# tusen-ai/SST

Hardware: AMD Instinct MI355X
Metric: LiDAR frames/sec (SST backbone fwd+bwd) at Waymo 0.32m voxels (higher is better)
Workload: dtype f32 (storage, accumulation, attention, LayerNorm, reductions: fp32; the dense products of the encoder layers from the EXACT three-way bf16 split of both fp32 operands, six bf16 MFMA products with fp32 accumulation - error vs float64 <= 2 x the fp32 matrix pipe's: tests/test_gpu_dense_f32x6.py)

## Files before the change

### include/sst_amd.h

```cpp
#ifndef SST_AMD_H
#define SST_AMD_H

#include <stdint.h>

#ifdef __cplusplus
extern "C" {
#endif

#define SST_OK 0
#define SST_ERR_ARG (-1)
#define SST_ERR_UNSUPPORTED (-2)
#define SST_ERR_KEYSPACE (-3)

typedef enum { SST_REDUCE_SUM = 0, SST_REDUCE_MEAN = 1, SST_REDUCE_MAX = 2 } sst_reduce_t;

const char* sst_version(void);

int sst_dynamic_voxelize_f32(const float* d_points, int64_t n, int64_t row_stride,
                             const float voxel_size[3], const float coors_range[6],
                             int32_t* d_coors, int64_t coors_stride, int coors_col0, int batch_idx,
                             void* stream);
void sst_dynamic_voxelize_grid(const float voxel_size[3], const float coors_range[6], int32_t grid_xyz[3]);

int64_t sst_scan_workspace_bytes(int64_t n);
int sst_exclusive_scan_i32(const int32_t* d_in, int32_t* d_out, int64_t n, int32_t* d_total,
                           void* d_workspace, void* stream);

int64_t sst_sort_workspace_bytes(int64_t n);
int sst_sort_pairs_u64(uint64_t* d_keys_in, uint64_t* d_keys_out, uint32_t* d_perm_out, int64_t n,
                       int key_bits, void* d_workspace, void* stream);

int64_t sst_unique_workspace_bytes(int64_t n);
int sst_unique_rows(const void* d_coors, int coor_is_i64, int64_t n, int ncols, int64_t row_stride,
                    const int64_t* h_mins, const int64_t* h_extents, int invalid_if_negative,
                    uint32_t* d_perm, int32_t* d_inverse, int32_t* d_offsets, uint64_t* d_ukeys,
                    int32_t* d_num_unique, void* d_workspace, void* stream);
int sst_unpack_keys(const uint64_t* d_ukeys, int64_t m, int ncols, const int64_t* h_mins,
                    const int64_t* h_extents, void* d_rows_out, int out_is_i64, int64_t out_stride,
                    int out_col0, void* stream);

int sst_segment_reduce_fwd_f32(const float* d_feats, int64_t n, int c, const uint32_t* d_perm,
                               const int32_t* d_offsets, const int32_t* d_group_index, int64_t m, int mode,
                               float* d_out, int32_t* d_argmax, const int32_t* d_m_limit, void* stream);
int64_t sst_segment_reduce_work_words(int64_t n, int64_t m, int c);
int sst_segment_reduce_fwd_work_f32(const float* d_feats, int64_t n, int c, const uint32_t* d_perm,
                                    const int32_t* d_offsets, const int32_t* d_group_index, int64_t m, int mode,
                                    float* d_out, int32_t* d_argmax, const int32_t* d_m_limit, int32_t* d_work,
                                    int64_t work_capacity, const float* d_scale, const float* d_shift, void* stream);
int64_t sst_segment_long_scratch_bytes(int64_t n, int64_t m, int c);
int sst_segment_reduce_long_f32(const float* d_feats, int64_t n, int c, const uint32_t* d_perm, const int32_t* d_inverse,
                                int inverse_shift, const int32_t* d_offsets, int64_t m, int mode, void* d_scratch,
                                float* d_out, int32_t* d_argmax, void* stream);
int sst_segment_reduce_profile_next(void* start, void* stop);
int sst_segment_reduce_bwd_f32(const float* d_grad_out, int64_t m, int c, const int32_t* d_inverse,
                               int inverse_shift, const int32_t* d_offsets, const int32_t* d_group_index,
                               const int32_t* d_argmax, int64_t n, int mode, float* d_grad_feats,
                               const int32_t* d_m_limit, void* stream);

int sst_concat_gather_f32(const float* d_x, int64_t ldx, int c1, const float* d_g, int64_t ldg, int c2,
                          const int32_t* d_idx, int64_t n, float* d_out, void* stream);

int sst_recover_bev_f32(const float* d_feats, int64_t ldf, const void* d_coors, int coor_is_i64, int64_t ldc, int64_t m,
                        int batch, int ny, int nx, int c, int32_t* d_cell_map, int32_t* d_cell_of_voxel, float* d_canvas,
                        void* stream);
int sst_recover_bev_bwd_f32(const float* d_grad_canvas, const int32_t* d_cell_of_voxel, int64_t m, int c,
                            float* d_grad_feats, void* stream);

int sst_vfe_decorate_f32(const float* d_points, int64_t ldp, int64_t n, int c, const int32_t* d_inverse,
                         const float* d_voxel_mean, int64_t ldm, float cluster_div, const void* d_coors,
                         int coor_is_i64, int64_t ldc, const float* voxel_size, const float* offsets,
                         int with_cluster, int with_center, float* d_out, int64_t ldo, void* stream);

int64_t sst_ingroup_rank_workspace_bytes(int64_t n);
int sst_ingroup_rank_i64(const int64_t* d_group, int64_t n, int key_bits, int64_t* d_rank,
                         void* d_workspace, void* stream);

int sst_window_coors(const void* d_coors, int coor_is_i64, int64_t m, const int32_t sparse_shape[3],
                     const int32_t window_shape[3], int32_t* d_win0, int32_t* d_ciw0,
                     int32_t* d_win1, int32_t* d_ciw1, void* stream);

int64_t sst_region_batching_workspace_bytes(int64_t m);
int sst_region_batching(const int32_t* d_win0, const int32_t* d_win1, int64_t m, int win_bits,
                        const int32_t* h_levels , int n_levels,
                        int32_t* d_keep, int32_t* d_newidx,
                        int32_t* d_level0, int32_t* d_level1, int32_t* d_inner0, int32_t* d_inner1,
                        int32_t* d_flat2win0, int32_t* d_flat2win1,
                        int32_t* d_tok0, int32_t* d_tok1, int32_t* d_winoff0, int32_t* d_winoff1,
                        int32_t* d_winlevel0, int32_t* d_winlevel1, int32_t* d_counts,
                        void* d_workspace, void* stream);
int sst_window_order_i32(const int32_t* d_winoff, int n_windows, int max_tokens, int32_t* d_order, void* stream);


int64_t sst_frame_windows_per_sample(const int32_t grid_zyx[3], const int32_t window_shape[3]);
int sst_frame_voxels_i32(const uint64_t* d_ukeys, const int32_t* d_inverse, const int32_t* d_num_groups, int64_t n_points, int batch_size, const int32_t grid_zyx[3],
                         int drop_mode, int32_t* d_vcoors, int32_t* d_gidx, int32_t* d_coors_map, int32_t* d_grid,
                         int32_t* d_counts, int32_t* d_dropped_groups, void* stream);
int64_t sst_window_plan_workspace_bytes(int64_t n_upper, int64_t n_windows);
int sst_window_plan_i32(const int32_t* d_vcoors, const int32_t* d_grid, int64_t n_upper, int batch_size,
                        const int32_t grid_zyx[3], const int32_t window_shape[3], const int32_t* h_levels, int n_levels,
                        uint32_t seed, int64_t* d_feat_index, int32_t* d_feat_index32, int64_t* d_out_coors,
                        int32_t* d_tok1, int32_t* d_winoff0, int32_t* d_winoff1, int32_t* d_posidx0, int32_t* d_posidx1,
                        int32_t* d_counts, void* d_workspace, void* stream);

int sst_sra_attn_fwd_f32(const float* d_q, const float* d_k, const float* d_v, int64_t ldq, int64_t ldk,
                         int64_t ldv, const int32_t* d_tok, const int32_t* d_winoff, int64_t n_windows,
                         int n_heads, float scale, int max_tokens, int impl, float* d_o, int64_t ldo,
                         float* d_lse, void* stream);
int64_t sst_sra_attn_bwd_workspace_bytes(int64_t n_tokens, int n_heads);
int sst_sra_attn_bwd_f32(const float* d_q, const float* d_k, const float* d_v, const float* d_o,
                         const float* d_do, const float* d_lse, int64_t ldq, int64_t ldk, int64_t ldv,
                         int64_t ldo, int64_t lddo, const int32_t* d_tok, const int32_t* d_winoff,
                         int64_t n_windows, int64_t n_tokens, int n_heads, float scale, int max_tokens,
                         int impl, float* d_dq, float* d_dk, float* d_dv, int64_t lddq, int64_t lddk,
                         int64_t lddv, void* d_workspace, void* stream);

int sst_sra_attn_fwd_ord_f32(const float* d_q, const float* d_k, const float* d_v, int64_t ldq, int64_t ldk, int64_t ldv,
                             const int32_t* d_tok, const int32_t* d_winoff, const int32_t* d_win_order, int64_t n_windows,
                             int n_heads, float scale, int max_tokens, int impl, float* d_o, int64_t ldo, float* d_lse,
                             void* stream);
int sst_sra_attn_bwd_ord_f32(const float* d_q, const float* d_k, const float* d_v, const float* d_o, const float* d_do,
                             const float* d_lse, int64_t ldq, int64_t ldk, int64_t ldv, int64_t ldo, int64_t lddo,
                             const int32_t* d_tok, const int32_t* d_winoff, const int32_t* d_win_order, int64_t n_windows,
                             int64_t n_tokens, int n_heads, float scale, int max_tokens, int impl, float* d_dq,
                             float* d_dk, float* d_dv, int64_t lddq, int64_t lddk, int64_t lddv, void* d_workspace,
                             void* stream);

int sst_sra_attn_cos_fwd_f32(const float* d_q, const float* d_k, const float* d_v, int64_t ldq, int64_t ldk, int64_t ldv,
                             const int32_t* d_tok, const int32_t* d_winoff, const int32_t* d_win_order, int64_t n_windows,
                             int n_heads, const float* d_head_scale, int max_tokens, float* d_o, int64_t ldo, float* d_lse,
                             void* stream);
int sst_sra_attn_cos_bwd_f32(const float* d_q, const float* d_k, const float* d_v, const float* d_o, const float* d_do,
                             const float* d_lse, int64_t ldq, int64_t ldk, int64_t ldv, int64_t ldo, int64_t lddo,
                             const int32_t* d_tok, const int32_t* d_winoff, const int32_t* d_win_order, int64_t n_windows,
                             int64_t n_tokens, int n_heads, const float* d_head_scale, int max_tokens, float* d_dq, float* d_dk,
                             float* d_dv, int64_t lddq, int64_t lddk, int64_t lddv, float* d_r, void* stream);

int sst_sra_attn_fwd_bf16(const void* d_q, const void* d_k, const void* d_v, int64_t ldq, int64_t ldk, int64_t ldv,
                          const int32_t* d_tok, const int32_t* d_winoff, int64_t n_windows, int n_heads, float scale,
                          int max_tokens, void* d_o, int64_t ldo, float* d_lse, void* stream);
int sst_sra_attn_bwd_bf16(const void* d_q, const void* d_k, const void* d_v, const void* d_o, const void* d_do,
                          const float* d_lse, int64_t ldq, int64_t ldk, int64_t ldv, int64_t ldo, int64_t lddo,
                          const int32_t* d_tok, const int32_t* d_winoff, int64_t n_windows, int n_heads, float scale,
                          int max_tokens, void* d_dq, void* d_dk, void* d_dv, int64_t lddq, int64_t lddk, int64_t lddv,
                          void* stream);
int sst_sra_attn_bf16_profile_next(int backward, void* start, void* stop);
int sst_sra_attn_fwd_ord_bf16(const void* d_q, const void* d_k, const void* d_v, int64_t ldq, int64_t ldk, int64_t ldv,
                              const int32_t* d_tok, const int32_t* d_winoff, const int32_t* d_win_order, int64_t n_windows,
                              int n_heads, float scale, int max_tokens, void* d_o, int64_t ldo, float* d_lse,
                              void* stream);
int sst_sra_attn_bwd_ord_bf16(const void* d_q, const void* d_k, const void* d_v, const void* d_o, const void* d_do,
                              const float* d_lse, int64_t ldq, int64_t ldk, int64_t ldv, int64_t ldo, int64_t lddo,
                              const int32_t* d_tok, const int32_t* d_winoff, const int32_t* d_win_order, int64_t n_windows,
                              int n_heads, float scale, int max_tokens, void* d_dq, void* d_dk, void* d_dv, int64_t lddq,
                              int64_t lddk, int64_t lddv, void* stream);
int sst_sra_attn_cos_fwd_bf16(const void* d_q, const void* d_k, const void* d_v, int64_t ldq, int64_t ldk, int64_t ldv,
                              const int32_t* d_tok, const int32_t* d_winoff, const int32_t* d_win_order, int64_t n_windows,
                              int n_heads, const float* d_head_scale, int max_tokens, void* d_o, int64_t ldo, float* d_lse,
                              void* stream);
int sst_sra_attn_cos_bwd_bf16(const void* d_q, const void* d_k, const void* d_v, const void* d_o, const void* d_do,
                              const float* d_lse, int64_t ldq, int64_t ldk, int64_t ldv, int64_t ldo, int64_t lddo,
                              const int32_t* d_tok, const int32_t* d_winoff, const int32_t* d_win_order, int64_t n_windows,
                              int n_heads, const float* d_head_scale, int max_tokens, void* d_dq, void* d_dk, void* d_dv,
                              int64_t lddq, int64_t lddk, int64_t lddv, float* d_r, void* stream);

int sst_add_layernorm_fwd_bf16(const void* d_x, const void* d_res, const float* d_weight, const float* d_bias, int64_t m,
                               int c, float eps, void* d_y, void* d_sum, float* d_stats, const float* d_pos_table,
                               const int32_t* d_pos_idx, void* d_y_plus_pos, void* stream);
int sst_add_layernorm_bwd_bf16(const void* d_dy, const void* d_dy2, const void* d_sum, const float* d_stats,
                               const float* d_weight, int64_t m, int c, void* d_dx, float* d_dweight, float* d_dbias,
                               void* d_workspace, void* stream);
int sst_cast_add_pos_bf16(const void* d_x, int x_is_bf16, int64_t m, int c, const float* d_pos_table,
                          const int32_t* d_pos_idx, void* d_out, void* stream);

int sst_tall_linear_bf16(const void* d_x, int64_t ldx, const void* d_w, const float* d_bias, int64_t m, int k, int n,
                         int epilogue, const void* d_aux_in, void* d_aux_out, int64_t ldaux, void* d_y, int64_t ldy,
                         void* stream);
int sst_tall_linear_bf16_partition(int64_t m, int k, int n, int epi_is_ln, int64_t* blocks, int64_t* rows_per_wave);
int sst_tall_linear_ln_bf16(const void* d_x, int64_t ldx, const void* d_w, const float* d_bias, int64_t m, int k,
                            const void* d_res, int64_t ldres, const float* d_ln_weight, const float* d_ln_bias, float eps,
                            void* d_y, void* d_sum, float* d_stats, const float* d_pos_table, const int32_t* d_pos_idx,
                            void* d_y_plus_pos, void* stream);
typedef struct sst_wgrad_problem_bf16 {
  const void* a;
  const void* b;
  int64_t lda, ldb, m;
// ... 12 lines not shown
int sst_cast_group_bf16(const sst_cast_problem_bf16* problems, int n, void* stream);

int sst_gather_rows_f32(const float* d_src, int64_t ld_src, const int32_t* d_idx, int64_t n_out, int c,
                        float fill, float* d_out, int64_t ld_out, void* stream);
int sst_add_table_rows_f32(const float* d_x, int64_t ldx, const float* d_table, int64_t ld_table, const int32_t* d_idx, int64_t m,
                           int c, float* d_out, int64_t ld_out, void* stream);
int sst_scatter_rows_f32(const float* d_src, int64_t ld_src, const int32_t* d_idx, int64_t n_src, int c,
                         float* d_out, int64_t ld_out, void* stream);

int sst_add_layernorm_act_fwd_f32(const float* d_x, const float* d_res, const float* d_weight, const float* d_bias,
                                  int64_t m, int c, float eps, int act, float* d_y, float* d_sum, float* d_stats,
                                  void* stream);
int sst_add_layernorm_act_bwd_f32(const float* d_dy, const float* d_sum, const float* d_stats, const float* d_weight,
                                  const float* d_bias, int act, int64_t m, int c, float* d_dx, float* d_dweight,
                                  float* d_dbias, void* d_workspace, void* stream);
int sst_add_layernorm_fwd_f32(const float* d_x, const float* d_res, const float* d_weight, const float* d_bias,
                              int64_t m, int c, float eps, float* d_y, float* d_sum, float* d_stats,
                              void* stream);
int sst_add_layernorm_pos_fwd_f32(const float* d_x, const float* d_res, const float* d_weight, const float* d_bias, int64_t m,
                                  int c, float eps, float* d_y, float* d_sum, float* d_stats, const float* d_pos_table,
                                  const int32_t* d_pos_idx, float* d_y_plus_pos, void* stream);
int64_t sst_add_layernorm_bwd_workspace_bytes(int64_t m, int c);
int sst_add_layernorm_bwd_f32(const float* d_dy, const float* d_sum, const float* d_stats,
                              const float* d_weight, int64_t m, int c, float* d_dx, float* d_dweight,
                              float* d_dbias, void* d_workspace, void* stream);
int64_t sst_colsum_workspace_bytes(int64_t m, int c);
int sst_colsum_f32(const float* d_x, int64_t m, int c, int64_t ld, float* d_out, void* d_workspace, void* stream);

int64_t sst_weight_grad_workspace_bytes(int64_t m, int out, int in);
int sst_weight_grad_f32(const float* d_dy, const float* d_x, int64_t m, int out, int in, int64_t ld_dy,
                        int64_t ld_x, float* d_dw, float* d_db, void* d_workspace, void* stream);
typedef struct sst_wgrad_problem_f32 {
  const float* dy;
  const float* x;
  int64_t m, ld_dy, ld_x;
  float* dw;
  float* db;
  int32_t out, in;
  const float* x_add_rows;
  const int32_t* x_add_index;
} sst_wgrad_problem_f32;
int64_t sst_weight_grad_group_workspace_bytes(const sst_wgrad_problem_f32* problems, int n);
int sst_weight_grad_group_f32(const sst_wgrad_problem_f32* problems, int n, void* d_workspace, void* stream);
int64_t sst_weight_grad_group_f32x6_workspace_bytes(const sst_wgrad_problem_f32* problems, int n);
int sst_weight_grad_group_f32x6(const sst_wgrad_problem_f32* problems, int n, void* d_workspace, void* stream);
int sst_weight_grad_group_f32x6_plan(const sst_wgrad_problem_f32* problems, int n, int* tiles, int* slices,
                                     int64_t* tokens_per_slice, int* lean_slices);

int64_t sst_bn_workspace_bytes(int64_t n, int c);
int sst_bn_stats_f32(const float* d_x, int64_t n, int c, int64_t ld, float* d_mean, float* d_var,
                     void* d_workspace, void* stream);
int sst_bn_act_fwd_f32(const float* d_x, int64_t n, int c, int64_t ldx, const float* d_scale,
                       const float* d_shift, int act, float* d_y, int64_t ldy, void* stream);
int sst_bn_act_bwd_reduce_f32(const float* d_dy, const float* d_x, int64_t n, int c, int64_t lddy, int64_t ldx,
                              const float* d_mean, const float* d_invstd, const float* d_scale,
                              const float* d_shift, int act, float* d_sum_g, float* d_sum_gxhat,
                              void* d_workspace, void* stream);
int sst_bn_act_bwd_apply_f32(const float* d_dy, const float* d_x, int64_t n, int c, int64_t lddy, int64_t ldx,
                             const float* d_mean, const float* d_invstd, const float* d_scale,
                             const float* d_shift, const float* d_coef_a, const float* d_coef_b, float coef_scale,
                             int act, float* d_dx, int64_t lddx, void* stream);
int sst_bn_prepare_f32(const float* d_x, int64_t n, int c, int64_t ld, const float* d_weight, const float* d_bias,
                       float eps, float* d_running_mean, float* d_running_var, float factor, float* d_out4,
                       void* d_workspace, void* stream);
int sst_bn_prepare_tracked_f32(const float* d_x, int64_t n, int c, int64_t ld, const float* d_weight,
                               const float* d_bias, float eps, float* d_running_mean, float* d_running_var,
                               float factor, int64_t* d_num_batches_tracked, float* d_out4, void* d_workspace,
                               void* stream);
int sst_vfe_linear_moments_f32(const float* d_x, int64_t ldx, int64_t n, int k, const float* d_w, int64_t ldw, int c,
                               float* d_y, int64_t ldy, void* d_workspace, void* stream);
int sst_bn_prepare_from_partials_f32(int64_t n, int c, const float* d_weight, const float* d_bias, float eps,
                                     float* d_running_mean, float* d_running_var, float factor,
                                     int64_t* d_num_batches_tracked, float* d_out4, void* d_workspace, void* stream);
int sst_bn_stats_from_partials_f32(int64_t n, int c, float* d_mean, float* d_var, void* d_workspace, void* stream);
int sst_bn_act_pool_bwd_reduce_f32(const float* d_dy, const float* d_x, int64_t n, int c, int64_t lddy, int64_t ldx,
                                   const float* d_mean, const float* d_invstd, const float* d_scale, const float* d_shift,
                                   int act, const int32_t* d_group, const int32_t* d_arg, const float* d_dpool, int64_t ldp,
                                   float* d_sum_g, float* d_sum_gxhat, void* d_workspace, void* stream);
int sst_bn_act_pool_bwd_apply_f32(const float* d_dy, const float* d_x, int64_t n, int c, int64_t lddy, int64_t ldx,
                                  const float* d_mean, const float* d_invstd, const float* d_scale, const float* d_shift,
                                  const float* d_coef_a, const float* d_coef_b, float coef_scale, int act,
                                  const int32_t* d_group, const int32_t* d_arg, const float* d_dpool, int64_t ldp, float* d_dx,
                                  int64_t lddx, void* stream);
int sst_bn_act_res_fwd_f32(const float* d_x, int64_t n, int c, int64_t ldx, const float* d_res, int64_t ldr,
                           const float* d_scale, const float* d_shift, int act, float* d_y, int64_t ldy, void* stream);
int sst_bn_act_res_bwd_reduce_f32(const float* d_dy, const float* d_x, const float* d_res, int64_t n, int c,
                                  int64_t lddy, int64_t ldx, int64_t ldr, const float* d_mean, const float* d_invstd,
                                  const float* d_scale, const float* d_shift, int act, float* d_sum_g,
                                  float* d_sum_gxhat, void* d_workspace, void* stream);
int sst_bn_act_res_bwd_apply_f32(const float* d_dy, const float* d_x, const float* d_res, int64_t n, int c,
                                 int64_t lddy, int64_t ldx, int64_t ldr, const float* d_mean, const float* d_invstd,
                                 const float* d_scale, const float* d_shift, const float* d_coef_a,
                                 const float* d_coef_b, float coef_scale, int act, float* d_dres, int64_t lddres,
                                 float* d_dx, int64_t lddx, void* stream);

int sst_tall_linear_f32(const float* d_x, int64_t ldx, const float* d_w, int64_t ldw, const float* d_bias,
                        int64_t m, int n, int k, int trans_w, int accumulate, float* d_y, int64_t ldy,
                        void* stream);
int sst_tall_linear_ln_f32(const float* d_x, int64_t ldx, const float* d_w, int64_t ldw, const float* d_bias, int64_t m, int k,
                           const float* d_res, int64_t ldres, const float* d_ln_weight, const float* d_ln_bias, float eps,
                           float* d_y, float* d_sum, float* d_stats, const float* d_pos_table, const int32_t* d_pos_idx,
                           float* d_y_plus_pos, void* stream);
int sst_tall_linear_epi_f32x3(const float* d_x, int64_t ldx, const float* d_w, int64_t ldw, int trans_w, const float* d_bias,
                              int64_t m, int k, int n, int epilogue, const float* d_aux_in, float* d_aux_out, int64_t ldaux,
                              float* d_y, int64_t ldy, void* stream);
int sst_tall_linear_ln_f32x3(const float* d_x, int64_t ldx, const float* d_w, int64_t ldw, const float* d_bias, int64_t m, int k,
                             const float* d_res, int64_t ldres, const float* d_ln_weight, const float* d_ln_bias, float eps,
                             float* d_y, float* d_sum, float* d_stats, const float* d_pos_table, const int32_t* d_pos_idx,
                             float* d_y_plus_pos, void* stream);
int sst_tall_linear_epi_f32x6(const float* d_x, int64_t ldx, const float* d_w, int64_t ldw, int trans_w, const float* d_bias,
                              int64_t m, int k, int n, int epilogue, const float* d_aux_in, float* d_aux_out, int64_t ldaux,
                              float* d_y, int64_t ldy, void* stream);
int sst_tall_linear_epi2_f32x6(const float* d_x, const float* d_x2, int x2_from_col, int64_t ldx, const float* d_w, int64_t ldw,
                               int trans_w, const float* d_bias, int64_t m, int k, int n, int epilogue, const float* d_aux_in,
                               float* d_aux_out, int64_t ldaux, float* d_y, int64_t ldy, void* stream);
int sst_tall_linear_add_rows_f32x6(const float* d_x, int64_t ldx, const float* d_w, int64_t ldw, int64_t m, int k, int n,
                                   const float* d_rows, int64_t ldrows, const int32_t* d_row_index, float* d_y, int64_t ldy,
                                   void* stream);
int sst_inproj_pos_f32x6(const float* d_x, int64_t ldx, const float* d_rows, const int32_t* d_index, const float* d_w, int64_t ldw,
                         const float* d_bias, int64_t m, float* d_y, int64_t ldy, void* stream);
int sst_tall_linear_f32x6_partition(int64_t m, int groups, int64_t* row_blocks, int64_t* rows_per_wave);
int sst_tall_linear_ln_f32x6(const float* d_x, int64_t ldx, const float* d_w, int64_t ldw, const float* d_bias, int64_t m, int k,
                             const float* d_res, int64_t ldres, const float* d_ln_weight, const float* d_ln_bias, float eps,
                             float* d_y, float* d_sum, float* d_stats, const float* d_pos_table, const int32_t* d_pos_idx,
                             float* d_y_plus_pos, void* stream);
int sst_add_layernorm_bwd2_f32(const float* d_dy, const float* d_dy2, const float* d_sum, const float* d_stats,
                               const float* d_weight, int64_t m, int c, float* d_dx, float* d_dweight, float* d_dbias,
                               void* d_workspace, void* stream);
typedef struct sst_encoder_layer_fwd_args {
  int64_t m, n_windows;
  int32_t n_heads, act, max_tokens, impl;
  float eps, scale;
  const float *x, *xp;
  const float *w_in, *b_in, *w_out, *b_out, *w1, *b1, *w2, *b2, *n1w, *n1b, *n2w, *n2b;
  const int32_t *tok, *winoff, *order;
  const float* pos_table;
  const int32_t* pos_idx;
  float *qkv, *o, *lse, *y1, *s1, *st1, *pre, *h, *s2, *y2, *st2, *y2p;
  const float* head_scale;
  void* wpack;
  const float* xpos_table;
  const int32_t* xpos_idx;
} sst_encoder_layer_fwd_args;
typedef struct sst_encoder_layer_bwd_args {
  int64_t m, n_windows;
  int32_t n_heads, act, max_tokens, impl;
  float eps, scale;
  const float *dy2, *dy2p;
  const float *x, *xp, *qkv, *o, *lse, *s1, *st1, *y1, *pre, *h, *s2, *st2;
  const float *w_in, *w_out, *w1, *w2, *n1w, *n2w;
  const int32_t *tok, *winoff, *order;
  float *ds2, *dpre, *ds1, *d_o, *dqkv;
  float *dw_in, *db_in, *dwo, *dbo, *dw1, *db1, *dw2, *db2, *dn1w, *dn1b, *dn2w, *dn2b;
  void* workspace;
  const float* head_scale;
  float* cos_r;
  float* dy1;
  const void* wpack;
  const float* xpos_table;
  const int32_t* xpos_idx;
} sst_encoder_layer_bwd_args;
int64_t sst_encoder_layer_bwd_workspace_bytes(int64_t m, int n_heads);
int64_t sst_encoder_layer_wpack_bytes(void);
int sst_encoder_layer_fwd_f32x6(const sst_encoder_layer_fwd_args* args, void* stream);
int sst_encoder_layer_bwd_f32x6(const sst_encoder_layer_bwd_args* args, void* stream);

// ... 733 lines not shown
```

### sst_amd/_lib.py

```python
import ctypes
import os
import subprocess

import torch

_HERE = os.path.dirname(os.path.abspath(__file__))
_CSRC = os.path.join(_HERE, 'csrc')
LIB_PATH = os.path.join(_CSRC, 'libsst_amd.so')

_lib = None

c_i64 = ctypes.c_int64
c_i32 = ctypes.c_int
c_f32 = ctypes.c_float
c_ptr = ctypes.c_void_p



class WgradProblemBF16(ctypes.Structure):
    _fields_ = [('a', c_ptr), ('b', c_ptr), ('lda', c_i64), ('ldb', c_i64), ('m', c_i64), ('out_w', c_ptr),
                ('out_b', c_ptr), ('p', ctypes.c_int32), ('bias_side', ctypes.c_int32),
                ('transpose_out', ctypes.c_int32), ('reserved', ctypes.c_int32)]


# ... 102 lines not shown
    + [(k, _I32 * 4) for k in ('q_inc', 'q_lo', 'q_hi')]
    + [('q_tag', ctypes.c_float * 4), ('lo', ctypes.c_float * 3), ('vs', ctypes.c_float * 3), ('grid', _I32 * 3)]))
IncrDeltaArgs = _struct('IncrDeltaArgs', 'sst_incr_delta_args of include/sst_amd.h', (
    [('base', ctypes.c_void_p * 8), ('n_base', c_i64 * 8), ('ld_base', c_i64 * 8), ('query', ctypes.c_void_p),
     ('n_query', c_i64), ('ld_query', c_i64), ('mask', ctypes.c_void_p), ('workspace', ctypes.c_void_p),
     ('workspace_bytes', c_i64), ('n_clouds', _I32), ('lower_bound', _I32), ('lo', ctypes.c_float * 3),
     ('vs', ctypes.c_float * 3), ('grid', _I32 * 3)]))
FrameTransformArgs = _struct('FrameTransformArgs', 'sst_frame_transform_args of include/sst_amd.h', (
    [('src', ctypes.c_void_p * 8), ('dst', ctypes.c_void_p * 8), ('n', c_i64 * 8), ('mat', (ctypes.c_float * 12) * 8),
     ('n_clouds', _I32), ('cols', _I32)]))
AugmentParams = _struct('AugmentParams', 'sst_augment_params of include/sst_amd.h', (
    [(k, _I32) for k in ('flip_h', 'flip_v', 'rotate', 'shuffle')]
    + [(k, ctypes.c_float) for k in ('cos', 'sin', 'scale', 'angle')]
    + [('trans', ctypes.c_float * 3), ('reserved', ctypes.c_float), ('range', ctypes.c_float * 6), ('seed', ctypes.c_uint64)]))
AugmentArgs = _struct('AugmentArgs', 'sst_augment_args of include/sst_amd.h', (
    [(k, ctypes.c_void_p) for k in ('points', 'row_offsets', 'n_pasted', 'block_offsets', 'params', 'planes', 'plane_offsets',
                                    'out', 'counts', 'workspace')]
    + [(k, c_i64) for k in ('workspace_bytes', 'n_total')]
    + [(k, _I32) for k in ('batch', 'cols', 'n_blocks', 'n_planes', 'norm_mask', 'reserved')]
    + [('norm_mean', ctypes.c_float * 8), ('norm_std', ctypes.c_float * 8)]))
AugmentBoxArgs = _struct('AugmentBoxArgs', 'sst_augment_box_args of include/sst_amd.h', (
    [(k, ctypes.c_void_p) for k in ('boxes', 'labels', 'box_offsets', 'params', 'boxes_out', 'labels_out', 'counts')]
    + [(k, _I32) for k in ('batch', 'cols', 'n_boxes', 'filter', 'always_rotate', 'reserved')]))
FgGroupOffsets = _struct('FgGroupOffsets', 'sst_fg_group_offsets of include/sst_amd.h', [('off', c_i64 * 33)])

_P = ctypes.c_void_p
EncoderLayerFwdArgs = _struct('EncoderLayerFwdArgs', 'sst_encoder_layer_fwd_args of include/sst_amd.h', (
    [('m', c_i64), ('n_windows', c_i64)] + [(k, ctypes.c_int32) for k in ('n_heads', 'act', 'max_tokens', 'impl')]
    + [('eps', ctypes.c_float), ('scale', ctypes.c_float)]
    + [(k, _P) for k in ('x', 'xp', 'w_in', 'b_in', 'w_out', 'b_out', 'w1', 'b1', 'w2', 'b2', 'n1w', 'n1b', 'n2w', 'n2b',
                         'tok', 'winoff', 'order', 'pos_table', 'pos_idx',
                         'qkv', 'o', 'lse', 'y1', 's1', 'st1', 'pre', 'h', 's2', 'y2', 'st2', 'y2p', 'head_scale', 'wpack',
                         'xpos_table', 'xpos_idx')]))
EncoderLayerBwdArgs = _struct('EncoderLayerBwdArgs', 'sst_encoder_layer_bwd_args of include/sst_amd.h', (
    [('m', c_i64), ('n_windows', c_i64)] + [(k, ctypes.c_int32) for k in ('n_heads', 'act', 'max_tokens', 'impl')]
    + [('eps', ctypes.c_float), ('scale', ctypes.c_float)]
    + [(k, _P) for k in ('dy2', 'dy2p', 'x', 'xp', 'qkv', 'o', 'lse', 's1', 'st1', 'y1', 'pre', 'h', 's2', 'st2',
                         'w_in', 'w_out', 'w1', 'w2', 'n1w', 'n2w', 'tok', 'winoff', 'order',
                         'ds2', 'dpre', 'ds1', 'd_o', 'dqkv',
                         'dw_in', 'db_in', 'dwo', 'dbo', 'dw1', 'db1', 'dw2', 'db2', 'dn1w', 'dn1b', 'dn2w', 'dn2b',
                         'workspace', 'head_scale', 'cos_r', 'dy1', 'wpack', 'xpos_table', 'xpos_idx')]))


EncoderTailFwdArgs = _struct('EncoderTailFwdArgs', 'sst_encoder_tail_fwd_args of include/sst_amd.h', (
    [('m', c_i64), ('act', ctypes.c_int32), ('reserved', ctypes.c_int32), ('eps', ctypes.c_float), ('reserved_f', ctypes.c_float)]
    + [(k, _P) for k in ('o', 'x', 'packed', 'b_out', 'b1', 'b2', 'n1w', 'n1b', 'n2w', 'n2b', 'pos_table', 'pos_idx',
                         's1', 'st1', 'y1', 'pre', 'h', 's2', 'st2', 'y2', 'y2p')]))
EncoderTailBwdArgs = _struct('EncoderTailBwdArgs', 'sst_encoder_tail_bwd_args of include/sst_amd.h', (
    [('m', c_i64), ('act', ctypes.c_int32), ('reserved', ctypes.c_int32)]
    + [(k, _P) for k in ('dy2', 'dy2p', 's2', 'st2', 'pre', 's1', 'st1', 'packed', 'n1w', 'n2w',
                         'ds2', 'dpre', 'ds1', 'd_o', 'dn2w', 'dn2b', 'dn1w', 'dn1b', 'workspace')]))

EncoderTailFwdBF16Args = _struct('EncoderTailFwdBF16Args', 'sst_encoder_tail_fwd_bf16_args of include/sst_amd.h', (
    [('m', c_i64), ('act', ctypes.c_int32), ('reserved', ctypes.c_int32), ('eps', ctypes.c_float), ('reserved_f', ctypes.c_float)]
    + [(k, _P) for k in ('o', 'x', 'packed', 'b_out', 'b1', 'b2', 'n1w', 'n1b', 'n2w', 'n2b', 'pos_table', 'pos_idx',
                         's1', 'st1', 'y1', 'pre', 'h', 's2', 'st2', 'y2', 'y2p')]))
EncoderTailBwdBF16Args = _struct('EncoderTailBwdBF16Args', 'sst_encoder_tail_bwd_bf16_args of include/sst_amd.h', (
    [('m', c_i64), ('act', ctypes.c_int32), ('reserved', ctypes.c_int32)]
    + [(k, _P) for k in ('dy2', 'dy2p', 's2', 'st2', 'pre', 's1', 'st1', 'packed', 'n1w', 'n2w',
                         'ds2', 'dpre', 'ds1', 'd_o', 'dn2w', 'dn2b', 'dn1w', 'dn1b', 'workspace')]))


EncoderLayerFwdBF16Args = _struct('EncoderLayerFwdBF16Args', 'sst_encoder_layer_fwd_bf16_args of include/sst_amd.h', (
    [('m', c_i64), ('n_windows', c_i64)] + [(k, ctypes.c_int32) for k in ('n_heads', 'act', 'max_tokens', 'reserved')]
    + [('eps', ctypes.c_float), ('scale', ctypes.c_float)]
    + [(k, _P) for k in ('x', 'xp', 'wqk', 'wv', 'wout', 'w1', 'w2', 'b_in', 'b_out', 'b1', 'b2', 'n1w', 'n1b', 'n2w', 'n2b',
                         'tok', 'winoff', 'order', 'pos_table', 'pos_idx',
                         'qk', 'v', 'o', 'lse', 'y1', 's1', 'st1', 'pre', 'h', 's2', 'st2', 'y2', 'y2p', 'head_scale', 'wpack')]))
EncoderLayerBwdBF16Args = _struct('EncoderLayerBwdBF16Args', 'sst_encoder_layer_bwd_bf16_args of include/sst_amd.h', (
    [('m', c_i64), ('n_windows', c_i64)] + [(k, ctypes.c_int32) for k in ('n_heads', 'act', 'max_tokens', 'reserved')]
    + [('eps', ctypes.c_float), ('scale', ctypes.c_float)]
    + [(k, _P) for k in ('dy2', 'dy2p', 'x', 'xp', 'qk', 'v', 'o', 'lse', 's1', 'st1', 'y1', 'pre', 'h', 's2', 'st2',
                         'wqk_t', 'wv_t', 'wout_t', 'w1_t', 'w2_t', 'n1w', 'n2w', 'tok', 'winoff', 'order',
                         'ds2', 'dpre', 'dy1', 'ds1', 'd_o', 'dqkv', 'dxp', 'dx',
                         'dw_in', 'db_in', 'dwo', 'dbo', 'dw1', 'db1', 'dw2', 'db2', 'dn1w', 'dn1b', 'dn2w', 'dn2b',
                         'workspace', 'head_scale', 'cos_r', 'wpack')]))


_SIGNATURES = {
    'sst_version': (ctypes.c_char_p, []),
    'sst_dynamic_voxelize_f32': (c_i32, [c_ptr, c_i64, c_i64, c_ptr, c_ptr, c_ptr, c_i64, c_i32, c_i32, c_ptr]),
    'sst_dynamic_voxelize_grid': (None, [c_ptr, c_ptr, c_ptr]),
    'sst_scan_workspace_bytes': (c_i64, [c_i64]),
    'sst_exclusive_scan_i32': (c_i32, [c_ptr, c_ptr, c_i64, c_ptr, c_ptr, c_ptr]),
    'sst_sort_workspace_bytes': (c_i64, [c_i64]),
    'sst_sort_pairs_u64': (c_i32, [c_ptr, c_ptr, c_ptr, c_i64, c_i32, c_ptr, c_ptr]),
    'sst_unique_workspace_bytes': (c_i64, [c_i64]),
    'sst_unique_rows': (c_i32, [c_ptr, c_i32, c_i64, c_i32, c_i64, c_ptr, c_ptr, c_i32,
                                c_ptr, c_ptr, c_ptr, c_ptr, c_ptr, c_ptr, c_ptr]),
    'sst_unpack_keys': (c_i32, [c_ptr, c_i64, c_i32, c_ptr, c_ptr, c_ptr, c_i32, c_i64, c_i32, c_ptr]),
    'sst_segment_reduce_fwd_f32': (c_i32, [c_ptr, c_i64, c_i32, c_ptr, c_ptr, c_ptr, c_i64, c_i32, c_ptr, c_ptr,
                                           c_ptr, c_ptr]),
    'sst_encoder_layer_bwd_workspace_bytes': (c_i64, [c_i64, c_i32]),
    'sst_tall_linear_f32x6_partition': (c_i32, [c_i64, c_i32, c_ptr, c_ptr]),
    'sst_inproj_pos_f32x6': (c_i32, [c_ptr, c_i64, c_ptr, c_ptr, c_ptr, c_i64, c_ptr, c_i64, c_ptr, c_i64, c_ptr]),
    'sst_encoder_layer_wpack_bytes': (c_i64, []),
    'sst_encoder_layer_fwd_f32x6': (c_i32, [c_ptr, c_ptr]),
    'sst_encoder_layer_bwd_f32x6': (c_i32, [c_ptr, c_ptr]),
    'sst_encoder_tail_pack_bytes': (c_i64, []),
    'sst_encoder_tail_pack_f32x6': (c_i32, [c_ptr, c_ptr, c_ptr, c_ptr, c_ptr]),
    'sst_encoder_tail_pack_f32x6_many': (c_i32, [c_ptr, c_ptr, c_ptr, c_ptr, c_i32, c_ptr]),
    'sst_encoder_tail_bwd_workspace_bytes': (c_i64, [c_i64]),
    'sst_encoder_tail_fwd_f32x6': (c_i32, [c_ptr, c_ptr]),
    'sst_encoder_tail_bwd_f32x6': (c_i32, [c_ptr, c_ptr]),
    'sst_encoder_tail_pack_bf16_bytes': (c_i64, []),
    'sst_encoder_tail_pack_bf16': (c_i32, [c_ptr, c_ptr, c_ptr, c_ptr, c_ptr]),
    'sst_encoder_tail_pack_bf16_many': (c_i32, [c_ptr, c_ptr, c_ptr, c_ptr, c_i32, c_ptr]),
    'sst_encoder_tail_bwd_bf16_workspace_bytes': (c_i64, [c_i64]),
    'sst_encoder_tail_fwd_bf16': (c_i32, [c_ptr, c_ptr]),
    'sst_encoder_tail_bwd_bf16': (c_i32, [c_ptr, c_ptr]),
    'sst_encoder_layer_bwd_bf16_workspace_bytes': (c_i64, [c_i64]),
    'sst_encoder_layer_fwd_bf16': (c_i32, [c_ptr, c_ptr]),
    'sst_encoder_layer_bwd_bf16': (c_i32, [c_ptr, c_ptr]),
    'sst_segment_reduce_work_words': (c_i64, [c_i64, c_i64, c_i32]),
    'sst_segment_reduce_fwd_work_f32': (c_i32, [c_ptr, c_i64, c_i32, c_ptr, c_ptr, c_ptr, c_i64, c_i32, c_ptr, c_ptr,
                                                c_ptr, c_ptr, c_i64, c_ptr, c_ptr, c_ptr]),
    'sst_vfe_linear_moments_f32': (c_i32, [c_ptr, c_i64, c_i64, c_i32, c_ptr, c_i64, c_i32, c_ptr, c_i64, c_ptr, c_ptr]),
    'sst_bn_prepare_from_partials_f32': (c_i32, [c_i64, c_i32, c_ptr, c_ptr, c_f32, c_ptr, c_ptr, c_f32, c_ptr, c_ptr, c_ptr,
                                                 c_ptr]),
    'sst_bn_stats_from_partials_f32': (c_i32, [c_i64, c_i32, c_ptr, c_ptr, c_ptr, c_ptr]),
    'sst_bn_act_pool_bwd_reduce_f32': (c_i32, [c_ptr, c_ptr, c_i64, c_i32, c_i64, c_i64, c_ptr, c_ptr, c_ptr, c_ptr, c_i32,
                                               c_ptr, c_ptr, c_ptr, c_i64, c_ptr, c_ptr, c_ptr, c_ptr]),
    'sst_bn_act_pool_bwd_apply_f32': (c_i32, [c_ptr, c_ptr, c_i64, c_i32, c_i64, c_i64, c_ptr, c_ptr, c_ptr, c_ptr, c_ptr,
                                              c_ptr, c_f32, c_i32, c_ptr, c_ptr, c_ptr, c_i64, c_ptr, c_i64, c_ptr]),
    'sst_tall_linear_add_rows_f32x6': (c_i32, [c_ptr, c_i64, c_ptr, c_i64, c_i64, c_i32, c_i32, c_ptr, c_i64, c_ptr, c_ptr,
                                               c_i64, c_ptr]),
    'sst_segment_long_scratch_bytes': (c_i64, [c_i64, c_i64, c_i32]),
    'sst_segment_reduce_long_f32': (c_i32, [c_ptr, c_i64, c_i32, c_ptr, c_ptr, c_i32, c_ptr, c_i64, c_i32, c_ptr, c_ptr, c_ptr,
                                            c_ptr]),
    'sst_segment_reduce_profile_next': (c_i32, [c_ptr, c_ptr]),
    'sst_segment_reduce_bwd_f32': (c_i32, [c_ptr, c_i64, c_i32, c_ptr, c_i32, c_ptr, c_ptr, c_ptr, c_i64, c_i32,
                                           c_ptr, c_ptr, c_ptr]),
    'sst_ingroup_rank_workspace_bytes': (c_i64, [c_i64]),
    'sst_ingroup_rank_i64': (c_i32, [c_ptr, c_i64, c_i32, c_ptr, c_ptr, c_ptr]),
    'sst_window_coors': (c_i32, [c_ptr, c_i32, c_i64, c_ptr, c_ptr, c_ptr, c_ptr, c_ptr, c_ptr, c_ptr]),
    'sst_window_order_i32': (c_i32, [c_ptr, c_i32, c_i32, c_ptr, c_ptr]),
    'sst_region_batching_workspace_bytes': (c_i64, [c_i64]),
    'sst_region_batching': (c_i32, [c_ptr, c_ptr, c_i64, c_i32, c_ptr, c_i32] + [c_ptr] * 15 + [c_ptr, c_ptr]),
    'sst_frame_windows_per_sample': (c_i64, [c_ptr, c_ptr]),
    'sst_frame_voxels_i32': (c_i32, [c_ptr, c_ptr, c_ptr, c_i64, c_i32, c_ptr, c_i32, c_ptr, c_ptr, c_ptr, c_ptr,
                                     c_ptr, c_ptr, c_ptr]),
    'sst_window_plan_workspace_bytes': (c_i64, [c_i64, c_i64]),
    'sst_window_plan_i32': (c_i32, [c_ptr, c_ptr, c_i64, c_i32, c_ptr, c_ptr, c_ptr, c_i32, ctypes.c_uint32] + [c_ptr] * 11),
    'sst_sra_attn_fwd_f32': (c_i32, [c_ptr, c_ptr, c_ptr, c_i64, c_i64, c_i64, c_ptr, c_ptr, c_i64, c_i32,
                                     c_f32, c_i32, c_i32, c_ptr, c_i64, c_ptr, c_ptr]),
    'sst_sra_attn_bwd_f32': (c_i32, [c_ptr] * 6 + [c_i64] * 5 + [c_ptr, c_ptr, c_i64, c_i64, c_i32, c_f32,
                                                                 c_i32, c_i32, c_ptr, c_ptr, c_ptr,
                                                                 c_i64, c_i64, c_i64, c_ptr, c_ptr]),
    'sst_sra_attn_fwd_ord_f32': (c_i32, [c_ptr, c_ptr, c_ptr, c_i64, c_i64, c_i64, c_ptr, c_ptr, c_ptr, c_i64, c_i32,
                                         c_f32, c_i32, c_i32, c_ptr, c_i64, c_ptr, c_ptr]),
    'sst_sra_attn_bwd_ord_f32': (c_i32, [c_ptr] * 6 + [c_i64] * 5 + [c_ptr, c_ptr, c_ptr, c_i64, c_i64, c_i32, c_f32,
                                                                     c_i32, c_i32, c_ptr, c_ptr, c_ptr,
                                                                     c_i64, c_i64, c_i64, c_ptr, c_ptr]),
    'sst_sra_attn_bwd_workspace_bytes': (c_i64, [c_i64, c_i32]),
    'sst_sra_attn_cos_fwd_f32': (c_i32, [c_ptr, c_ptr, c_ptr, c_i64, c_i64, c_i64, c_ptr, c_ptr, c_ptr, c_i64, c_i32,
                                         c_ptr, c_i32, c_ptr, c_i64, c_ptr, c_ptr]),
    'sst_sra_attn_cos_bwd_f32': (c_i32, [c_ptr] * 6 + [c_i64] * 5 + [c_ptr, c_ptr, c_ptr, c_i64, c_i64, c_i32, c_ptr,
                                                                     c_i32, c_ptr, c_ptr, c_ptr,
                                                                     c_i64, c_i64, c_i64, c_ptr, c_ptr]),
    'sst_sra_attn_fwd_bf16': (c_i32, [c_ptr, c_ptr, c_ptr, c_i64, c_i64, c_i64, c_ptr, c_ptr, c_i64, c_i32, c_f32, c_i32,
                                      c_ptr, c_i64, c_ptr, c_ptr]),
    'sst_sra_attn_bwd_bf16': (c_i32, [c_ptr] * 6 + [c_i64] * 5 + [c_ptr, c_ptr, c_i64, c_i32, c_f32, c_i32, c_ptr, c_ptr,
                                                                  c_ptr, c_i64, c_i64, c_i64, c_ptr]),
    'sst_sra_attn_bf16_profile_next': (c_i32, [c_i32, c_ptr, c_ptr]),
    'sst_sra_attn_fwd_ord_bf16': (c_i32, [c_ptr, c_ptr, c_ptr, c_i64, c_i64, c_i64, c_ptr, c_ptr, c_ptr, c_i64, c_i32, c_f32,
                                          c_i32, c_ptr, c_i64, c_ptr, c_ptr]),
    'sst_sra_attn_bwd_ord_bf16': (c_i32, [c_ptr] * 6 + [c_i64] * 5 + [c_ptr, c_ptr, c_ptr, c_i64, c_i32, c_f32, c_i32, c_ptr,
                                                                      c_ptr, c_ptr, c_i64, c_i64, c_i64, c_ptr]),
    'sst_sra_attn_cos_fwd_bf16': (c_i32, [c_ptr, c_ptr, c_ptr, c_i64, c_i64, c_i64, c_ptr, c_ptr, c_ptr, c_i64, c_i32, c_ptr,
                                          c_i32, c_ptr, c_i64, c_ptr, c_ptr]),
    'sst_sra_attn_cos_bwd_bf16': (c_i32, [c_ptr] * 6 + [c_i64] * 5 + [c_ptr, c_ptr, c_ptr, c_i64, c_i32, c_ptr, c_i32, c_ptr,
                                                                      c_ptr, c_ptr, c_i64, c_i64, c_i64, c_ptr, c_ptr]),
    'sst_add_layernorm_fwd_bf16': (c_i32, [c_ptr, c_ptr, c_ptr, c_ptr, c_i64, c_i32, c_f32, c_ptr, c_ptr, c_ptr, c_ptr,
                                           c_ptr, c_ptr, c_ptr]),
    'sst_add_layernorm_bwd_bf16': (c_i32, [c_ptr, c_ptr, c_ptr, c_ptr, c_ptr, c_i64, c_i32, c_ptr, c_ptr, c_ptr, c_ptr,
                                           c_ptr]),
    'sst_cast_add_pos_bf16': (c_i32, [c_ptr, c_i32, c_i64, c_i32, c_ptr, c_ptr, c_ptr, c_ptr]),
    'sst_weight_grad_group_workspace_bytes': (c_i64, [c_ptr, c_i32]),
    'sst_weight_grad_group_f32': (c_i32, [c_ptr, c_i32, c_ptr, c_ptr]),
    'sst_weight_grad_group_f32x6_workspace_bytes': (c_i64, [c_ptr, c_i32]),
    'sst_weight_grad_group_f32x6': (c_i32, [c_ptr, c_i32, c_ptr, c_ptr]),
    'sst_weight_grad_group_f32x6_plan': (c_i32, [c_ptr, c_i32, c_ptr, c_ptr, c_ptr, c_ptr]),
    'sst_tall_linear_ln_f32': (c_i32, [c_ptr, c_i64, c_ptr, c_i64, c_ptr, c_i64, c_i32, c_ptr, c_i64, c_ptr, c_ptr, c_f32, c_ptr,
                                       c_ptr, c_ptr, c_ptr, c_ptr, c_ptr, c_ptr]),
    'sst_tall_linear_ln_f32x3': (c_i32, [c_ptr, c_i64, c_ptr, c_i64, c_ptr, c_i64, c_i32, c_ptr, c_i64, c_ptr, c_ptr, c_f32, c_ptr,
                                         c_ptr, c_ptr, c_ptr, c_ptr, c_ptr, c_ptr]),
    'sst_tall_linear_epi_f32x3': (c_i32, [c_ptr, c_i64, c_ptr, c_i64, c_i32, c_ptr, c_i64, c_i32, c_i32, c_i32, c_ptr, c_ptr,
                                          c_i64, c_ptr, c_i64, c_ptr]),
    'sst_tall_linear_ln_f32x6': (c_i32, [c_ptr, c_i64, c_ptr, c_i64, c_ptr, c_i64, c_i32, c_ptr, c_i64, c_ptr, c_ptr, c_f32, c_ptr,
                                         c_ptr, c_ptr, c_ptr, c_ptr, c_ptr, c_ptr]),
    'sst_tall_linear_epi_f32x6': (c_i32, [c_ptr, c_i64, c_ptr, c_i64, c_i32, c_ptr, c_i64, c_i32, c_i32, c_i32, c_ptr, c_ptr,
                                          c_i64, c_ptr, c_i64, c_ptr]),
    'sst_tall_linear_epi2_f32x6': (c_i32, [c_ptr, c_ptr, c_i32, c_i64, c_ptr, c_i64, c_i32, c_ptr, c_i64, c_i32, c_i32, c_i32,
                                           c_ptr, c_ptr, c_i64, c_ptr, c_i64, c_ptr]),
    'sst_add_layernorm_bwd2_f32': (c_i32, [c_ptr, c_ptr, c_ptr, c_ptr, c_ptr, c_i64, c_i32, c_ptr, c_ptr, c_ptr, c_ptr, c_ptr]),
    'sst_tall_linear_epi_f32': (c_i32, [c_ptr, c_i64, c_ptr, c_i64, c_i32, c_ptr, c_i64, c_i32, c_i32, c_i32, c_ptr, c_ptr,
                                        c_i64, c_ptr, c_i64, c_ptr]),
    'sst_tall_linear_bf16': (c_i32, [c_ptr, c_i64, c_ptr, c_ptr, c_i64, c_i32, c_i32, c_i32, c_ptr, c_ptr, c_i64, c_ptr,
                                     c_i64, c_ptr]),
    'sst_tall_linear_bf16_partition': (c_i32, [c_i64, c_i32, c_i32, c_i32, c_ptr, c_ptr]),
    'sst_tall_linear_ln_bf16': (c_i32, [c_ptr, c_i64, c_ptr, c_ptr, c_i64, c_i32, c_ptr, c_i64, c_ptr, c_ptr, c_f32, c_ptr, c_ptr,
                                        c_ptr, c_ptr, c_ptr, c_ptr, c_ptr]),
    'sst_wgrad_group_workspace_bytes': (c_i64, [c_ptr, c_i32]),
    'sst_wgrad_group_bf16': (c_i32, [c_ptr, c_i32, c_ptr, c_ptr]),
    'sst_cast_group_bf16': (c_i32, [c_ptr, c_i32, c_ptr]),
    'sst_gather_rows_f32': (c_i32, [c_ptr, c_i64, c_ptr, c_i64, c_i32, c_f32, c_ptr, c_i64, c_ptr]),
    'sst_add_table_rows_f32': (c_i32, [c_ptr, c_i64, c_ptr, c_i64, c_ptr, c_i64, c_i32, c_ptr, c_i64, c_ptr]),
    'sst_scatter_rows_f32': (c_i32, [c_ptr, c_i64, c_ptr, c_i64, c_i32, c_ptr, c_i64, c_ptr]),
    'sst_add_layernorm_fwd_f32': (c_i32, [c_ptr, c_ptr, c_ptr, c_ptr, c_i64, c_i32, c_f32, c_ptr, c_ptr, c_ptr,
                                          c_ptr]),
    'sst_add_layernorm_bwd_workspace_bytes': (c_i64, [c_i64, c_i32]),
    'sst_add_layernorm_pos_fwd_f32': (c_i32, [c_ptr, c_ptr, c_ptr, c_ptr, c_i64, c_i32, c_f32, c_ptr, c_ptr, c_ptr, c_ptr, c_ptr,
                                              c_ptr, c_ptr]),
    'sst_add_layernorm_act_fwd_f32': (c_i32, [c_ptr, c_ptr, c_ptr, c_ptr, c_i64, c_i32, c_f32, c_i32, c_ptr, c_ptr, c_ptr,
                                              c_ptr]),
    'sst_add_layernorm_act_bwd_f32': (c_i32, [c_ptr, c_ptr, c_ptr, c_ptr, c_ptr, c_i32, c_i64, c_i32, c_ptr, c_ptr, c_ptr,
                                              c_ptr, c_ptr]),
    'sst_add_layernorm_bwd_f32': (c_i32, [c_ptr, c_ptr, c_ptr, c_ptr, c_i64, c_i32, c_ptr, c_ptr, c_ptr, c_ptr,
                                          c_ptr]),
    'sst_weight_grad_workspace_bytes': (c_i64, [c_i64, c_i32, c_i32]),
    'sst_weight_grad_f32': (c_i32, [c_ptr, c_ptr, c_i64, c_i32, c_i32, c_i64, c_i64, c_ptr, c_ptr, c_ptr, c_ptr]),
    'sst_colsum_workspace_bytes': (c_i64, [c_i64, c_i32]),
    'sst_colsum_f32': (c_i32, [c_ptr, c_i64, c_i32, c_i64, c_ptr, c_ptr, c_ptr]),
    'sst_tall_linear_f32': (c_i32, [c_ptr, c_i64, c_ptr, c_i64, c_ptr, c_i64, c_i32, c_i32, c_i32, c_i32, c_ptr, c_i64,
                                    c_ptr]),
    'sst_tall_linear_gelu_f32': (c_i32, [c_ptr, c_i64, c_ptr, c_i64, c_ptr, c_i64, c_i32, c_i32, c_i32, c_i32, c_ptr, c_ptr,
# ... 319 lines not shown
```

### sst_amd/csrc/bn.hip

```cpp
#include "common.h"

namespace {

constexpr int kBnThreads = 256;

struct bn_pool_grad {
  const int32_t* group;
  const int32_t* arg;
  const float* dpool;
  int64_t ldp;
};
__device__ __forceinline__ float4 bn_pool_part(const bn_pool_grad& pg, int64_t row, int c, int cc) {
  float4 g = make_float4(0.f, 0.f, 0.f, 0.f);
  const int v = pg.group[row];
  if (v >= 0) {
    const int4 a = *(const int4*)(pg.arg + (int64_t)v * c + cc * 4);
    const float4 d = *(const float4*)(pg.dpool + (int64_t)v * pg.ldp + cc * 4);
    g.x = a.x == (int)row ? d.x : 0.f;
    g.y = a.y == (int)row ? d.y : 0.f;
    g.z = a.z == (int)row ? d.z : 0.f;
    g.w = a.w == (int)row ? d.w : 0.f;
  }
  return g;
}
// ... 134 lines not shown
    out[3 * c + ch] = sh;
    if (running_mean != nullptr) running_mean[ch] = (1.f - factor) * running_mean[ch] + factor * mean;
    if (running_var != nullptr) running_var[ch] = (1.f - factor) * running_var[ch] + factor * (var * unbiased);
    if (tracked != nullptr && ch == 0) tracked[0] += 1;
  }
}

__global__ __launch_bounds__(kBnThreads) void bn_act_fwd_k(const float* __restrict__ x, int64_t n, int c, int64_t ldx,
                                                          const float* __restrict__ scale,
                                                          const float* __restrict__ shift, int act,
                                                          const float* __restrict__ res, int64_t ldr,
                                                          float* __restrict__ y, int64_t ldy) {
  const int c4 = c >> 2;
  const int64_t total = n * c4;
  for (int64_t i = (int64_t)blockIdx.x * kBnThreads + threadIdx.x; i < total; i += (int64_t)gridDim.x * kBnThreads) {
    const int64_t row = i / c4;
    const int cc = (int)(i - row * c4);
    const float4 v = *(const float4*)(x + row * ldx + cc * 4);
    const float4 sc = *(const float4*)(scale + cc * 4);
    const float4 sh = *(const float4*)(shift + cc * 4);
    float4 o = make_float4(v.x * sc.x + sh.x, v.y * sc.y + sh.y, v.z * sc.z + sh.z, v.w * sc.w + sh.w);
    if (res != nullptr) {
      const float4 r = *(const float4*)(res + row * ldr + cc * 4);
      o.x += r.x, o.y += r.y, o.z += r.z, o.w += r.w;
    }
    if (act) {
      o.x = o.x > 0.f ? o.x : 0.f;
      o.y = o.y > 0.f ? o.y : 0.f;
      o.z = o.z > 0.f ? o.z : 0.f;
      o.w = o.w > 0.f ? o.w : 0.f;
    }
    *(float4*)(y + row * ldy + cc * 4) = o;
  }
}

__global__ __launch_bounds__(kBnThreads) void bn_act_bwd_k(const float* __restrict__ dy, const float* __restrict__ x,
                                                          int64_t n, int c, int64_t lddy, int64_t ldx,
                                                          const float* __restrict__ mean,
                                                          const float* __restrict__ invstd,
                                                          const float* __restrict__ scale,
                                                          const float* __restrict__ shift,
                                                          const float* __restrict__ ca, const float* __restrict__ cb,
                                                          float coef_scale, int act, const float* __restrict__ res,
                                                          int64_t ldr, float* __restrict__ dres, int64_t lddres,
                                                          float* __restrict__ dx, int64_t lddx, const bn_pool_grad pg) {
  const int c4 = c >> 2;
  const int64_t total = n * c4;
  for (int64_t i = (int64_t)blockIdx.x * kBnThreads + threadIdx.x; i < total; i += (int64_t)gridDim.x * kBnThreads) {
    const int64_t row = i / c4;
    const int cc = (int)(i - row * c4);
    const float4 v = *(const float4*)(x + row * ldx + cc * 4);
    float4 g = make_float4(0.f, 0.f, 0.f, 0.f);
    if (dy != nullptr) g = *(const float4*)(dy + row * lddy + cc * 4);
    if (pg.group != nullptr) {
      const float4 sp = bn_pool_part(pg, row, c, cc);
      g.x += sp.x, g.y += sp.y, g.z += sp.z, g.w += sp.w;
    }
    const float4 sc = *(const float4*)(scale + cc * 4);
    const float4 sh = *(const float4*)(shift + cc * 4);
    const float4 mu = *(const float4*)(mean + cc * 4);
    const float4 is = *(const float4*)(invstd + cc * 4);
    float4 a = *(const float4*)(ca + cc * 4);
    float4 b = *(const float4*)(cb + cc * 4);
    a.x *= coef_scale, a.y *= coef_scale, a.z *= coef_scale, a.w *= coef_scale;
    b.x *= coef_scale, b.y *= coef_scale, b.z *= coef_scale, b.w *= coef_scale;
    if (act) {
      float4 r = make_float4(0.f, 0.f, 0.f, 0.f);
      if (res != nullptr) r = *(const float4*)(res + row * ldr + cc * 4);
      g.x = (v.x * sc.x + sh.x + r.x) > 0.f ? g.x : 0.f;
      g.y = (v.y * sc.y + sh.y + r.y) > 0.f ? g.y : 0.f;
      g.z = (v.z * sc.z + sh.z + r.z) > 0.f ? g.z : 0.f;
      g.w = (v.w * sc.w + sh.w + r.w) > 0.f ? g.w : 0.f;
    }
    if (dres != nullptr) *(float4*)(dres + row * lddres + cc * 4) = g;
    float4 o;
    o.x = sc.x * (g.x - a.x - (v.x - mu.x) * is.x * b.x);
    o.y = sc.y * (g.y - a.y - (v.y - mu.y) * is.y * b.y);
    o.z = sc.z * (g.z - a.z - (v.z - mu.z) * is.z * b.z);
    o.w = sc.w * (g.w - a.w - (v.w - mu.w) * is.w * b.w);
    *(float4*)(dx + row * lddx + cc * 4) = o;
  }
}

__global__ __launch_bounds__(kBnThreads) void vfe_linear_smallk_k(const float* __restrict__ x, int64_t ldx, int64_t n, int k,
                                                                 const float* __restrict__ w, int64_t ldw, int c,
                                                                 float* __restrict__ y, int64_t ldy, int64_t rows_per_block,
                                                                 double* __restrict__ partial) {
  extern __shared__ __attribute__((aligned(16))) double red[];
  const int c4 = c >> 2;
  const int rpi = kBnThreads / c4;
  float* wt = (float*)(red + (size_t)rpi * 2 * c);
  for (int i = threadIdx.x; i < k * c; i += kBnThreads) {
    const int kk = i / c, ch = i - kk * c;
    wt[i] = w[(int64_t)ch * ldw + kk];
  }
  __syncthreads();
  const int ry = threadIdx.x / c4, cx = threadIdx.x - ry * c4;
  const int64_t beg = (int64_t)blockIdx.x * rows_per_block;
  const int64_t end = beg + rows_per_block < n ? beg + rows_per_block : n;
  double s1[4] = {0., 0., 0., 0.}, s2[4] = {0., 0., 0., 0.};
  if (ry < rpi) {
    for (int64_t row = beg + ry; row < end; row += rpi) {
      const float* xr = x + row * ldx;
      float4 acc = make_float4(0.f, 0.f, 0.f, 0.f);
      for (int kk = 0; kk < k; ++kk) {
        const float xv = xr[kk];
        const float4 wv = *(const float4*)(wt + kk * c + cx * 4);
        acc.x = fmaf(xv, wv.x, acc.x), acc.y = fmaf(xv, wv.y, acc.y), acc.z = fmaf(xv, wv.z, acc.z), acc.w = fmaf(xv, wv.w, acc.w);
      }
      *(float4*)(y + row * ldy + cx * 4) = acc;
      s1[0] += acc.x, s1[1] += acc.y, s1[2] += acc.z, s1[3] += acc.w;
      s2[0] += (double)acc.x * acc.x, s2[1] += (double)acc.y * acc.y;
      s2[2] += (double)acc.z * acc.z, s2[3] += (double)acc.w * acc.w;
    }
#pragma unroll
    for (int q = 0; q < 4; ++q) {
      red[(size_t)ry * 2 * c + cx * 4 + q] = s1[q];
      red[(size_t)ry * 2 * c + c + cx * 4 + q] = s2[q];
    }
  }
  __syncthreads();
  double* dst = partial + (int64_t)blockIdx.x * 2 * c;
  for (int i = threadIdx.x; i < 2 * c; i += kBnThreads) {
    double t = 0.;
    for (int r = 0; r < rpi; ++r) t += red[(size_t)r * 2 * c + i];
    dst[i] = t;
  }
}

int moments_grid(int64_t n, int64_t* rows_per_block) {
  int64_t rpb = 128;
  int64_t grid = sst_div_up(n, rpb);
  if (grid > 512) {
    rpb = sst_div_up(n, 512);
    grid = sst_div_up(n, rpb);
  }
  *rows_per_block = rpb;
  return (int)grid;
}

bool bn_shape_ok(int64_t n, int c) { return n >= 0 && c >= 4 && (c & 3) == 0 && c <= 1024; }

}

extern "C" {

int64_t sst_bn_workspace_bytes(int64_t n, int c) {
  (void)n;
  return (int64_t)1024 * 2 * c * sizeof(double) + 256;
}

int sst_bn_stats_f32(const float* d_x, int64_t n, int c, int64_t ld, float* d_mean, float* d_var, void* d_workspace,
                     void* stream) {
  if (!bn_shape_ok(n, c) || ld < c || (ld & 3)) return SST_ERR_UNSUPPORTED;
  if (n == 0) return SST_ERR_ARG;
  if (!d_x || !d_mean || !d_var || !d_workspace || ((uintptr_t)d_x & 15)) return SST_ERR_ARG;
  hipStream_t st = (hipStream_t)stream;
  int64_t rpb;
  const int grid = moments_grid(n, &rpb);
  double* partial = (double*)d_workspace;
  const size_t lds = (size_t)kBnThreads * 8 * sizeof(double);
  hipLaunchKernelGGL(bn_moments_k<0>, dim3(grid), dim3(kBnThreads), lds, st, d_x, nullptr, n, c, ld, 0, nullptr,
                     nullptr, nullptr, nullptr, 0, nullptr, 0, rpb, partial, bn_pool_grad{nullptr, nullptr, nullptr, 0});
  hipLaunchKernelGGL(bn_finish_k<0>, dim3((c + 31) / 32), dim3(1024), 0, st, partial, grid, c, 1.0 / (double)n,
                     d_mean, d_var);
  SST_LAUNCH_CHECK();
// ... 129 lines not shown
  const int rpi = kBnThreads / (c >> 2);
  const size_t lds = (size_t)rpi * 2 * c * sizeof(double) + (size_t)k * c * sizeof(float);
  hipLaunchKernelGGL(vfe_linear_smallk_k, dim3(grid), dim3(kBnThreads), lds, (hipStream_t)stream, d_x, ldx, n, k, d_w, ldw, c,
                     d_y, ldy, rpb, (double*)d_workspace);
  SST_LAUNCH_CHECK();
  return SST_OK;
}

int sst_bn_prepare_from_partials_f32(int64_t n, int c, const float* d_weight, const float* d_bias, float eps,
                                     float* d_running_mean, float* d_running_var, float factor,
                                     int64_t* d_num_batches_tracked, float* d_out4, void* d_workspace, void* stream) {
  if (!bn_shape_ok(n, c)) return SST_ERR_UNSUPPORTED;
  if (n == 0 || !d_out4 || !d_workspace) return SST_ERR_ARG;
  int64_t rpb;
  const int grid = moments_grid(n, &rpb);
  const float unbiased = n > 1 ? (float)((double)n / (double)(n - 1)) : 1.f;
  hipLaunchKernelGGL(bn_prepare_finish_k, dim3((c + 31) / 32), dim3(1024), 0, (hipStream_t)stream, (const double*)d_workspace,
                     grid, c, 1.0 / (double)n, d_weight, d_bias, eps, d_running_mean, d_running_var, factor, unbiased,
                     d_num_batches_tracked, d_out4);
  SST_LAUNCH_CHECK();
  return SST_OK;
}

int sst_bn_stats_from_partials_f32(int64_t n, int c, float* d_mean, float* d_var, void* d_workspace, void* stream) {
  if (!bn_shape_ok(n, c)) return SST_ERR_UNSUPPORTED;
  if (n == 0 || !d_mean || !d_var || !d_workspace) return SST_ERR_ARG;
  int64_t rpb;
  const int grid = moments_grid(n, &rpb);
  hipLaunchKernelGGL(bn_finish_k<0>, dim3((c + 31) / 32), dim3(1024), 0, (hipStream_t)stream, (const double*)d_workspace, grid,
                     c, 1.0 / (double)n, d_mean, d_var);
  SST_LAUNCH_CHECK();
  return SST_OK;
}

int sst_bn_act_pool_bwd_reduce_f32(const float* d_dy, const float* d_x, int64_t n, int c, int64_t lddy, int64_t ldx,
                                   const float* d_mean, const float* d_invstd, const float* d_scale, const float* d_shift,
                                   int act, const int32_t* d_group, const int32_t* d_arg, const float* d_dpool, int64_t ldp,
                                   float* d_sum_g, float* d_sum_gxhat, void* d_workspace, void* stream) {
  if (!bn_shape_ok(n, c) || ldx < c || (ldx & 3) || act < 0 || act > 1 || ldp < c || (ldp & 3)) return SST_ERR_UNSUPPORTED;
  if (d_dy && (lddy < c || (lddy & 3) || ((uintptr_t)d_dy & 15))) return SST_ERR_UNSUPPORTED;
  if (!d_sum_g || !d_sum_gxhat) return SST_ERR_ARG;
  hipStream_t st = (hipStream_t)stream;
  if (n == 0) {
    SST_HIP(hipMemsetAsync(d_sum_g, 0, sizeof(float) * c, st));
    SST_HIP(hipMemsetAsync(d_sum_gxhat, 0, sizeof(float) * c, st));
    return SST_OK;
  }
  if (!d_x || !d_mean || !d_invstd || !d_scale || !d_shift || !d_workspace || !d_group || !d_arg || !d_dpool ||
      ((uintptr_t)d_x & 15) || ((uintptr_t)d_arg & 15) || ((uintptr_t)d_dpool & 15))
    return SST_ERR_ARG;
  int64_t rpb;
  const int grid = moments_grid(n, &rpb);
  double* partial = (double*)d_workspace;
  const size_t lds = (size_t)kBnThreads * 8 * sizeof(double);
  hipLaunchKernelGGL(bn_moments_k<1>, dim3(grid), dim3(kBnThreads), lds, st, d_x, d_dy, n, c, ldx, lddy, d_mean, d_invstd,
                     d_scale, d_shift, act, nullptr, 0, rpb, partial, bn_pool_grad{d_group, d_arg, d_dpool, ldp});
  hipLaunchKernelGGL(bn_finish_k<1>, dim3((c + 31) / 32), dim3(1024), 0, st, partial, grid, c, 0.0, d_sum_g, d_sum_gxhat);
  SST_LAUNCH_CHECK();
  return SST_OK;
}

int sst_bn_act_pool_bwd_apply_f32(const float* d_dy, const float* d_x, int64_t n, int c, int64_t lddy, int64_t ldx,
                                  const float* d_mean, const float* d_invstd, const float* d_scale, const float* d_shift,
                                  const float* d_coef_a, const float* d_coef_b, float coef_scale, int act,
                                  const int32_t* d_group, const int32_t* d_arg, const float* d_dpool, int64_t ldp, float* d_dx,
                                  int64_t lddx, void* stream) {
  if (!bn_shape_ok(n, c) || ldx < c || lddx < c || (ldx & 3) || (lddx & 3) || act < 0 || act > 1 || ldp < c || (ldp & 3))
    return SST_ERR_UNSUPPORTED;
  if (d_dy && (lddy < c || (lddy & 3) || ((uintptr_t)d_dy & 15))) return SST_ERR_UNSUPPORTED;
  if (n == 0) return SST_OK;
  if (!d_x || !d_mean || !d_invstd || !d_scale || !d_shift || !d_coef_a || !d_coef_b || !d_dx || !d_group || !d_arg ||
      !d_dpool || ((uintptr_t)d_x & 15) || ((uintptr_t)d_dx & 15) || ((uintptr_t)d_arg & 15) || ((uintptr_t)d_dpool & 15))
    return SST_ERR_ARG;
  const int64_t total = n * (c >> 2);
  int64_t grid = sst_div_up(total, kBnThreads);
  if (grid > 8192) grid = 8192;
  hipLaunchKernelGGL(bn_act_bwd_k, dim3((unsigned)grid), dim3(kBnThreads), 0, (hipStream_t)stream, d_dy, d_x, n, c, lddy, ldx,
                     d_mean, d_invstd, d_scale, d_shift, d_coef_a, d_coef_b, coef_scale, act, nullptr, 0, nullptr, 0, d_dx, lddx,
                     bn_pool_grad{d_group, d_arg, d_dpool, ldp});
  SST_LAUNCH_CHECK();
  return SST_OK;
}

}
```

### sst_amd/csrc/frame_plan.hip

```cpp
#include "common.h"

namespace {

struct fp_geom {
  int B, gz, gy, gx;
  int wx, wy, wz;
  int nwx, nwy, nwz;
  int sh[2][3];
  int n_levels;
  int cap[8], lo[8], hi[8];
};

__device__ __forceinline__ void fp_decode(uint64_t key, const fp_geom& G, int& b, int& z, int& y, int& x) {
  uint64_t k = key - 1;
  x = (int)(k % (uint64_t)(G.gx + 1)) - 1;
  k /= (uint64_t)(G.gx + 1);
  y = (int)(k % (uint64_t)(G.gy + 1)) - 1;
  k /= (uint64_t)(G.gy + 1);
  z = (int)(k % (uint64_t)(G.gz + 1)) - 1;
  b = (int)(k / (uint64_t)(G.gz + 1));
}

__device__ int fp_lower_bound(const uint64_t* __restrict__ ukeys, int m_all, uint64_t key) {
  int lo = 0, hi = m_all;
// ... 171 lines not shown
          const bool kp = vox[q] >= 0 && rank[q] < cap;
          const uint64_t bal = __ballot(kp);
          if (kp) inner[vox[q]] = run + __popcll(bal & lt);
          run += __popcll(bal);
        }
      }
    }
    if (lane == 0) cntk[w] = kept;
  }
}


__global__ __launch_bounds__(1024) void fp_window_scan_k(const int32_t* __restrict__ cntk0,
                                                         const int32_t* __restrict__ cntk1, int n_win,
                                                         int32_t* __restrict__ tokbase0, int32_t* __restrict__ tokbase1,
                                                         int32_t* __restrict__ winoff0, int32_t* __restrict__ winoff1,
                                                         int32_t* __restrict__ d_counts) {
  __shared__ int wsum[16], wsum2[16];
  __shared__ int smax;
  const int s = blockIdx.x;
  const int32_t* cnt = s ? cntk1 : cntk0;
  int32_t* tokbase = s ? tokbase1 : tokbase0;
  int32_t* winoff = s ? winoff1 : winoff0;
  const int tid = threadIdx.x, wave = tid >> 6, lane = tid & 63;
  if (tid == 0) smax = 0;
  int carry_tok = 0, carry_win = 0, my_max = 0;
  for (int base = 0; base < n_win; base += 1024) {
    const int w = base + tid;
    const int c = w < n_win ? cnt[w] : 0;
    const int ne = c > 0 ? 1 : 0;
    my_max = c > my_max ? c : my_max;
    const int ic = sst_wave_incl_scan(c);
    const int in = sst_wave_incl_scan(ne);
    if (lane == 63) {
      wsum[wave] = ic;
      wsum2[wave] = in;
    }
    __syncthreads();
    int off_c = 0, off_n = 0, tot_c = 0, tot_n = 0;
#pragma unroll
    for (int k = 0; k < 16; ++k) {
      const int a = wsum[k], bq = wsum2[k];
      if (k < wave) {
        off_c += a;
        off_n += bq;
      }
      tot_c += a;
      tot_n += bq;
    }
    __syncthreads();
    const int tb = carry_tok + off_c + ic - c;
    const int cw = carry_win + off_n + in - ne;
    if (w < n_win) {
      tokbase[w] = tb;
      if (ne) winoff[cw] = tb;
    }
    carry_tok += tot_c;
    carry_win += tot_n;
  }
  atomicMax(&smax, my_max);
  __syncthreads();
  if (tid == 0) {
    winoff[carry_win] = carry_tok;
    d_counts[2 + s] = carry_win;
    d_counts[4 + s] = smax;
    if (s == 0) d_counts[1] = carry_tok;
  }
}

__device__ __forceinline__ void fp_window_of(const fp_geom& G, int s, int b, int z, int y, int x, int& w, int& pos) {
  const int xs = x + G.sh[s][0], ys = y + G.sh[s][1], zs = z + G.sh[s][2];
  const int wxi = xs / G.wx, wyi = ys / G.wy, wzi = zs / G.wz;
  w = b * (G.nwx * G.nwy * G.nwz) + wxi * G.nwy * G.nwz + wyi * G.nwz + wzi;
  pos = ((zs - wzi * G.wz) * G.wy + (ys - wyi * G.wy)) * G.wx + (xs - wxi * G.wx);
}

__global__ __launch_bounds__(256) void fp_fill_k(const int32_t* __restrict__ vcoors, const int32_t* __restrict__ d_counts,
                                                 fp_geom G, const int32_t* __restrict__ keep,
                                                 const int32_t* __restrict__ inner0, const int32_t* __restrict__ inner1,
                                                 const int32_t* __restrict__ tokbase0,
                                                 const int32_t* __restrict__ tokbase1, int64_t* __restrict__ feat_index,
                                                 int32_t* __restrict__ feat_index32,
                                                 int64_t* __restrict__ out_coors, int32_t* __restrict__ tok1,
                                                 int32_t* __restrict__ posidx0, int32_t* __restrict__ posidx1) {
  const int m = d_counts[0];
  for (int v = blockIdx.x * blockDim.x + threadIdx.x; v < m; v += gridDim.x * blockDim.x) {
    if (keep[v] == 0) continue;
    const int b = vcoors[4 * v], z = vcoors[4 * v + 1], y = vcoors[4 * v + 2], x = vcoors[4 * v + 3];
    int w0, p0, w1, p1;
    fp_window_of(G, 0, b, z, y, x, w0, p0);
    fp_window_of(G, 1, b, z, y, x, w1, p1);
    const int ni = tokbase0[w0] + inner0[v];
    feat_index[ni] = v;
    feat_index32[ni] = v;
    out_coors[4 * (int64_t)ni + 0] = b;
    out_coors[4 * (int64_t)ni + 1] = z;
    out_coors[4 * (int64_t)ni + 2] = y;
    out_coors[4 * (int64_t)ni + 3] = x;
    posidx0[ni] = p0;
    posidx1[ni] = p1;
    tok1[tokbase1[w1] + inner1[v]] = ni;
  }
}

int fill_geom(fp_geom* G, int batch_size, const int32_t grid_zyx[3], const int32_t window_shape[3],
              const int32_t* h_levels, int n_levels) {
  if (batch_size < 1 || batch_size > 64 || !grid_zyx || !window_shape) return SST_ERR_ARG;
  G->B = batch_size;
  G->gz = grid_zyx[0];
  G->gy = grid_zyx[1];
  G->gx = grid_zyx[2];
  G->wx = window_shape[0];
  G->wy = window_shape[1];
  G->wz = window_shape[2];
  if (G->gz < 1 || G->gy < 1 || G->gx < 1 || G->wx < 1 || G->wy < 1 || G->wz < 1) return SST_ERR_ARG;
  if ((int64_t)G->wx * G->wy * G->wz > 512) return SST_ERR_UNSUPPORTED;
  if ((int64_t)G->B * G->gz * G->gy * G->gx > ((int64_t)1 << 28)) return SST_ERR_UNSUPPORTED;
  G->nwx = (G->gx + G->wx - 1) / G->wx + 1;
  G->nwy = (G->gy + G->wy - 1) / G->wy + 1;
  G->nwz = (G->gz + G->wz - 1) / G->wz + 1;
  G->sh[0][0] = G->wx;
  G->sh[0][1] = G->wy;
  G->sh[0][2] = G->wz;
  G->sh[1][0] = G->wx / 2;
  G->sh[1][1] = G->wy / 2;
  G->sh[1][2] = G->wz / 2;
  if (G->gz == G->wz) G->sh[0][2] = G->sh[1][2] = 0;
  G->n_levels = n_levels;
  for (int l = 0; l < 8; ++l) {
    G->cap[l] = (h_levels && l < n_levels) ? h_levels[3 * l + 0] : 0;
    G->lo[l] = (h_levels && l < n_levels) ? h_levels[3 * l + 1] : 0;
    G->hi[l] = (h_levels && l < n_levels) ? h_levels[3 * l + 2] : 0;
  }
  return SST_OK;
}

}

extern "C" {

int64_t sst_frame_windows_per_sample(const int32_t grid_zyx[3], const int32_t window_shape[3]) {
  fp_geom G;
  if (fill_geom(&G, 1, grid_zyx, window_shape, nullptr, 0) != SST_OK) return -1;
  return (int64_t)G.nwx * G.nwy * G.nwz;
}

int sst_frame_voxels_i32(const uint64_t* d_ukeys, const int32_t* d_inverse, const int32_t* d_num_groups, int64_t n_points, int batch_size, const int32_t grid_zyx[3],
                         int drop_mode, int32_t* d_vcoors, int32_t* d_gidx, int32_t* d_coors_map, int32_t* d_grid,
                         int32_t* d_counts, int32_t* d_dropped_groups, void* stream) {
  if (n_points < 0 || (drop_mode != 0 && drop_mode != 1)) return SST_ERR_ARG;
  const int32_t win1[3] = {1, 1, 1};
  fp_geom G;
  int rc = fill_geom(&G, batch_size, grid_zyx, win1, nullptr, 0);
  if (rc != SST_OK) return rc;
  if (!d_counts || !d_grid) return SST_ERR_ARG;
  hipStream_t st = (hipStream_t)stream;
  SST_HIP(hipMemsetAsync(d_counts, 0, 8 * sizeof(int32_t), st));
  SST_HIP(hipMemsetAsync(d_grid, 0xff, sizeof(int32_t) * (size_t)G.B * G.gz * G.gy * G.gx, st));
  if (d_dropped_groups) SST_HIP(hipMemsetAsync(d_dropped_groups, 0xff, sizeof(int32_t) * (size_t)G.B, st));
  if (n_points == 0) return SST_OK;
  if (!d_ukeys || !d_inverse || !d_num_groups || !d_vcoors || !d_gidx || !d_coors_map) return SST_ERR_ARG;
  if (n_points > 0x7fffffff) return SST_ERR_UNSUPPORTED;
  hipLaunchKernelGGL(fp_voxels_k, dim3(sst_grid_1d(n_points, 256)), dim3(256), 0, st, d_ukeys, d_inverse, (int)n_points,
                     d_num_groups, G, drop_mode, d_vcoors, d_gidx, d_coors_map, d_grid, d_counts, d_dropped_groups);
  SST_LAUNCH_CHECK();
  return SST_OK;
}

int64_t sst_window_plan_workspace_bytes(int64_t n_upper, int64_t n_windows) {
  const int64_t n = n_upper > 0 ? n_upper : 1, w = n_windows > 0 ? n_windows : 1;
  return 4 * sst_align_up(4 * n, 256) + 4 * sst_align_up(4 * (w + 1), 256);
}

int sst_window_plan_i32(const int32_t* d_vcoors, const int32_t* d_grid, int64_t n_upper, int batch_size,
                        const int32_t grid_zyx[3], const int32_t window_shape[3], const int32_t* h_levels, int n_levels,
                        uint32_t seed, int64_t* d_feat_index, int32_t* d_feat_index32, int64_t* d_out_coors,
                        int32_t* d_tok1,
                        int32_t* d_winoff0, int32_t* d_winoff1, int32_t* d_posidx0, int32_t* d_posidx1,
                        int32_t* d_counts, void* d_workspace, void* stream) {
  if (n_upper < 0 || n_levels < 1 || n_levels > 8 || !h_levels) return SST_ERR_ARG;
  fp_geom G;
  int rc = fill_geom(&G, batch_size, grid_zyx, window_shape, h_levels, n_levels);
  if (rc != SST_OK) return rc;
  if (n_upper == 0) return SST_OK;
  if (!d_vcoors || !d_grid || !d_feat_index || !d_feat_index32 || !d_out_coors || !d_tok1 || !d_winoff0 || !d_winoff1 || !d_posidx0 ||
      !d_posidx1 || !d_counts || !d_workspace)
    return SST_ERR_ARG;
  if (n_upper >= ((int64_t)1 << 30)) return SST_ERR_UNSUPPORTED;
  hipStream_t st = (hipStream_t)stream;
  const int n_win = G.B * G.nwx * G.nwy * G.nwz;
  sst_carver cv(d_workspace);
  int32_t* keep_a = cv.take<int32_t>(n_upper);
  int32_t* keep = cv.take<int32_t>(n_upper);
  int32_t* inner0 = cv.take<int32_t>(n_upper);
  int32_t* inner1 = cv.take<int32_t>(n_upper);
  int32_t* cntk0 = cv.take<int32_t>(n_win + 1);
  int32_t* cntk1 = cv.take<int32_t>(n_win + 1);
  int32_t* tokbase0 = cv.take<int32_t>(n_win + 1);
  int32_t* tokbase1 = cv.take<int32_t>(n_win + 1);
  SST_HIP(hipMemsetAsync(keep_a, 0, 2 * sst_align_up(4 * n_upper, 256), st));
  const dim3 wgrid((unsigned)((n_win + 3) / 4));
  hipLaunchKernelGGL(fp_window_pass_k<0>, wgrid, dim3(256), 0, st, d_grid, G, seed, (const int32_t*)nullptr, keep_a,
                     (int32_t*)nullptr, (int32_t*)nullptr);
  hipLaunchKernelGGL(fp_window_pass_k<1>, wgrid, dim3(256), 0, st, d_grid, G, seed, keep_a, keep, inner1, cntk1);
  hipLaunchKernelGGL(fp_window_pass_k<2>, wgrid, dim3(256), 0, st, d_grid, G, seed, keep, (int32_t*)nullptr, inner0,
                     cntk0);
  hipLaunchKernelGGL(fp_window_scan_k, dim3(2), dim3(1024), 0, st, cntk0, cntk1, n_win, tokbase0, tokbase1, d_winoff0,
                     d_winoff1, d_counts);
  hipLaunchKernelGGL(fp_fill_k, dim3(sst_grid_1d(n_upper, 256)), dim3(256), 0, st, d_vcoors, d_counts, G, keep, inner0,
                     inner1, tokbase0, tokbase1, d_feat_index, d_feat_index32, d_out_coors, d_tok1, d_posidx0, d_posidx1);
  SST_LAUNCH_CHECK();
  return SST_OK;
}

}
```

### sst_amd/csrc/sort_scan.hip

```cpp
#include "common.h"

namespace {

constexpr int kScanThreads = 256;
constexpr int kScanIpt = 8;
constexpr int kScanTile = kScanThreads * kScanIpt;

__device__ __forceinline__ int block_excl_scan_256(int v, int& total, int* lds) {
  const int incl = sst_wave_incl_scan(v);
  const int wave = threadIdx.x >> 6, lane = threadIdx.x & 63;
  if (lane == 63) lds[wave] = incl;
  __syncthreads();
  int woff = 0, tot = 0;
#pragma unroll
  for (int w = 0; w < 4; ++w) {
    const int s = lds[w];
    if (w < wave) woff += s;
    tot += s;
  }
  __syncthreads();
  total = tot;
  return woff + incl - v;
}

__global__ __launch_bounds__(kScanThreads) void scan_reduce_k(const int32_t* __restrict__ in,
                                                              int32_t* __restrict__ block_sums, int64_t n) {
  __shared__ int lds[4];
  const int64_t base = (int64_t)blockIdx.x * kScanTile + (int64_t)threadIdx.x * kScanIpt;
  int s = 0;
#pragma unroll
  for (int k = 0; k < kScanIpt; ++k) {
    const int64_t i = base + k;
    if (i < n) s += in[i];
  }
  int total;
  (void)block_excl_scan_256(s, total, lds);
  if (threadIdx.x == 0) block_sums[blockIdx.x] = total;
}

__global__ __launch_bounds__(kScanThreads) void scan_spine_k(int32_t* __restrict__ sums, int nb,
                                                             int32_t* __restrict__ total_out) {
  __shared__ int lds[4];
  int carry = 0;
  for (int base = 0; base < nb; base += kScanThreads) {
    const int i = base + threadIdx.x;
    const int v = (i < nb) ? sums[i] : 0;
    int total;
    const int ex = block_excl_scan_256(v, total, lds);
    if (i < nb) sums[i] = carry + ex;
    carry += total;
  }
  if (threadIdx.x == 0 && total_out != nullptr) *total_out = carry;
}

__global__ __launch_bounds__(kScanThreads) void scan_apply_k(const int32_t* in, int32_t* out,
                                                             const int32_t* __restrict__ block_offsets,
                                                             int64_t n) {
  __shared__ int lds[4];
  const int64_t base = (int64_t)blockIdx.x * kScanTile + (int64_t)threadIdx.x * kScanIpt;
  int v[kScanIpt];
  int s = 0;
#pragma unroll
  for (int k = 0; k < kScanIpt; ++k) {
    const int64_t i = base + k;
    v[k] = (i < n) ? in[i] : 0;
    s += v[k];
  }
  int total;
  int run = block_excl_scan_256(s, total, lds) + block_offsets[blockIdx.x];
#pragma unroll
  for (int k = 0; k < kScanIpt; ++k) {
    const int64_t i = base + k;
    if (i < n) out[i] = run;
    run += v[k];
  }
}

int scan_impl(const int32_t* d_in, int32_t* d_out, int64_t n, int32_t* d_total, void* ws, hipStream_t st) {
  if (n <= 0) {
    if (d_total) SST_HIP(hipMemsetAsync(d_total, 0, sizeof(int32_t), st));
    return SST_OK;
  }
  const int nb = (int)sst_div_up(n, kScanTile);
  int32_t* sums = (int32_t*)ws;
  hipLaunchKernelGGL(scan_reduce_k, dim3(nb), dim3(kScanThreads), 0, st, d_in, sums, n);
  hipLaunchKernelGGL(scan_spine_k, dim3(1), dim3(kScanThreads), 0, st, sums, nb, d_total);
  hipLaunchKernelGGL(scan_apply_k, dim3(nb), dim3(kScanThreads), 0, st, d_in, d_out, sums, n);
  SST_LAUNCH_CHECK();
  return SST_OK;
}

int64_t scan_ws_bytes(int64_t n) { return sst_align_up(4 * (sst_div_up(n > 0 ? n : 1, kScanTile) + 1), 256); }

constexpr int kRadixBits = 8;
constexpr int kRadix = 1 << kRadixBits;
constexpr int kSortThreads = 256;
constexpr int kSortIpt = 8;
constexpr int kSortTile = kSortThreads * kSortIpt;

__global__ __launch_bounds__(kSortThreads) void radix_hist_k(const uint64_t* __restrict__ keys, int64_t n,
                                                             int shift, int32_t* __restrict__ ghist,
                                                             int nblocks) {
  __shared__ int hist[kRadix];
  hist[threadIdx.x] = 0;
  __syncthreads();
  const int64_t base = (int64_t)blockIdx.x * kSortTile;
#pragma unroll
  for (int k = 0; k < kSortIpt; ++k) {
    const int64_t i = base + (int64_t)k * kSortThreads + threadIdx.x;
    if (i < n) atomicAdd(&hist[(int)((keys[i] >> shift) & (kRadix - 1))], 1);
  }
  __syncthreads();
  ghist[(int64_t)threadIdx.x * nblocks + blockIdx.x] = hist[threadIdx.x];
}

__global__ __launch_bounds__(kSortThreads) void radix_scatter_k(
    const uint64_t* __restrict__ keys_in, const uint32_t* __restrict__ vals_in,
    uint64_t* __restrict__ keys_out, uint32_t* __restrict__ vals_out, int64_t n, int shift,
    const int32_t* __restrict__ gscan, int nblocks) {
  __shared__ int wcount[4][kRadix];
  __shared__ int woff[4][kRadix];
  const int tid = threadIdx.x, wave = tid >> 6, lane = tid & 63;
#pragma unroll
  for (int w = 0; w < 4; ++w) wcount[w][tid] = 0;
  __syncthreads();

  const int64_t wbase = (int64_t)blockIdx.x * kSortTile + (int64_t)wave * (kSortIpt * 64);
  uint64_t key[kSortIpt];
  int rank[kSortIpt];
  const uint64_t lt_mask = (lane == 0) ? 0ull : (~0ull >> (64 - lane));
#pragma unroll
  for (int j = 0; j < kSortIpt; ++j) {
    const int64_t i = wbase + (int64_t)j * 64 + lane;
    const bool valid = i < n;
    key[j] = valid ? keys_in[i] : 0ull;
    const int d = (int)((key[j] >> shift) & (kRadix - 1));
    uint64_t peers = __ballot(valid);
#pragma unroll
    for (int b = 0; b < kRadixBits; ++b) {
      const bool bit = (d >> b) & 1;
      const uint64_t bal = __ballot(bit);
      peers &= bit ? bal : ~bal;
    }
    const int below = __popcll(peers & lt_mask);
    int prior = 0;
    if (valid) prior = wcount[wave][d];
    __builtin_amdgcn_wave_barrier();
    if (valid && below == 0) wcount[wave][d] = prior + __popcll(peers);
    __builtin_amdgcn_wave_barrier();
    rank[j] = prior + below;
  }
  __syncthreads();
  {
    int run = gscan[(int64_t)tid * nblocks + blockIdx.x];
#pragma unroll
    for (int w = 0; w < 4; ++w) {
      woff[w][tid] = run;
      run += wcount[w][tid];
    }
  }
  __syncthreads();
#pragma unroll
  for (int j = 0; j < kSortIpt; ++j) {
// ... 124 lines not shown
}

int fill_pack_params(int ncols, const int64_t* mins, const int64_t* extents, int invalid_if_negative,
                     pack_params* pp) {
  if (ncols < 1 || ncols > 8) return SST_ERR_ARG;
  pp->ncols = ncols;
  pp->invalid_if_negative = invalid_if_negative;
  const uint64_t limit = (uint64_t)1 << 62;
  uint64_t total = 1;
  for (int j = ncols - 1; j >= 0; --j) {
    if (extents[j] < 1) return SST_ERR_ARG;
    pp->mins[j] = mins[j];
    pp->extents[j] = extents[j];
    pp->strides[j] = (int64_t)total;
    if ((uint64_t)extents[j] > limit / total) return SST_ERR_KEYSPACE;
    total *= (uint64_t)extents[j];
  }
  uint64_t maxkey = total;
  int bits = 1;
  while (bits < 63 && (maxkey >> bits) != 0) ++bits;
  return bits;
}

__global__ void u64_from_i64_k(const int64_t* __restrict__ in, int64_t n, uint64_t* __restrict__ out) {
  for (int64_t i = (int64_t)blockIdx.x * blockDim.x + threadIdx.x; i < n; i += (int64_t)gridDim.x * blockDim.x)
    out[i] = (uint64_t)in[i];
}

__global__ void rank_from_sorted_k(const uint32_t* __restrict__ perm, const int32_t* __restrict__ inverse,
                                   const int32_t* __restrict__ offsets, int64_t n, int64_t* __restrict__ rank) {
  for (int64_t i = (int64_t)blockIdx.x * blockDim.x + threadIdx.x; i < n; i += (int64_t)gridDim.x * blockDim.x) {
    const uint32_t row = perm[i];
    rank[row] = (int64_t)i - (int64_t)offsets[inverse[row]];
  }
}

}

int sst_scan_i32_internal(const int32_t* d_in, int32_t* d_out, int64_t n, int32_t* d_total, void* ws,
                          hipStream_t st) {
  return scan_impl(d_in, d_out, n, d_total, ws, st);
}
int64_t sst_scan_ws_internal(int64_t n) { return scan_ws_bytes(n); }

int64_t sst_unique_ws_internal(int64_t n) {
  const int64_t nn = n > 0 ? n : 1;
  return 2 * sst_align_up(8 * nn, 256)
         + 2 * sst_align_up(4 * nn, 256)
         + 2 * sst_align_up(4 * nn, 256)
         + sort_ws_bytes(nn) + scan_ws_bytes(nn);
}

int sst_unique_keys_internal(uint64_t* keys, uint64_t* keys_alt, int64_t n, int key_bits, uint32_t* d_perm_out,
                             int32_t* d_inverse, int32_t* d_offsets, uint64_t* d_ukeys, int32_t* d_num_unique,
                             void* ws, hipStream_t st) {
  if (n <= 0) {
    SST_HIP(hipMemsetAsync(d_num_unique, 0, sizeof(int32_t), st));
    SST_HIP(hipMemsetAsync(d_offsets, 0, sizeof(int32_t), st));
    return SST_OK;
  }
  sst_carver cv(ws);
  uint32_t* pa = cv.take<uint32_t>(n);
  uint32_t* pb = cv.take<uint32_t>(n);
  int32_t* flags = cv.take<int32_t>(n);
  int32_t* excl = cv.take<int32_t>(n);
  void* sort_ws = (void*)cv.take<char>(sort_ws_bytes(n));
  void* scan_ws = (void*)cv.take<char>(scan_ws_bytes(n));
  sort_result sr;
  int rc = sort_impl(keys, keys_alt, pa, pb, n, key_bits, sort_ws, st, &sr);
  if (rc != SST_OK) return rc;
  const int grid = sst_grid_1d(n, 256);
  hipLaunchKernelGGL(head_flags_k, dim3(grid), dim3(256), 0, st, sr.keys, n, flags);
  rc = scan_impl(flags, excl, n, nullptr, scan_ws, st);
  if (rc != SST_OK) return rc;
  hipLaunchKernelGGL(unique_finish_k, dim3(grid), dim3(256), 0, st, sr.keys, sr.perm, flags, excl, n, d_inverse,
                     d_offsets, d_ukeys, d_perm_out, d_num_unique);
  SST_LAUNCH_CHECK();
  return SST_OK;
}

extern "C" {

int64_t sst_scan_workspace_bytes(int64_t n) { return scan_ws_bytes(n); }

int sst_exclusive_scan_i32(const int32_t* d_in, int32_t* d_out, int64_t n, int32_t* d_total, void* d_workspace,
                           void* stream) {
  if (n < 0 || (n > 0 && (!d_in || !d_out || !d_workspace))) return SST_ERR_ARG;
  return scan_impl(d_in, d_out, n, d_total, d_workspace, (hipStream_t)stream);
}

int64_t sst_sort_workspace_bytes(int64_t n) { return sort_ws_bytes(n > 0 ? n : 1) + sst_align_up(4 * (n > 0 ? n : 1), 256); }

int sst_sort_pairs_u64(uint64_t* d_keys_in, uint64_t* d_keys_out, uint32_t* d_perm_out, int64_t n, int key_bits,
                       void* d_workspace, void* stream) {
  if (n < 0 || key_bits < 1 || key_bits > 64) return SST_ERR_ARG;
  if (n == 0) return SST_OK;
  if (!d_keys_in || !d_keys_out || !d_perm_out || !d_workspace) return SST_ERR_ARG;
  hipStream_t st = (hipStream_t)stream;
  sst_carver cv(d_workspace);
  uint32_t* p_tmp = cv.take<uint32_t>(n);
  void* sort_ws = (void*)cv.take<char>(sort_ws_bytes(n));
  const int passes = (key_bits + kRadixBits - 1) / kRadixBits;
  sort_result sr;
  int rc;
  if (passes & 1) {
    rc = sort_impl(d_keys_in, d_keys_out, d_perm_out, p_tmp, n, key_bits, sort_ws, st, &sr);
  } else {
    SST_HIP(hipMemcpyAsync(d_keys_out, d_keys_in, sizeof(uint64_t) * n, hipMemcpyDeviceToDevice, st));
    rc = sort_impl(d_keys_out, d_keys_in, p_tmp, d_perm_out, n, key_bits, sort_ws, st, &sr);
  }
  if (rc != SST_OK) return rc;
  if (sr.keys != d_keys_out || sr.perm != d_perm_out) return SST_ERR_UNSUPPORTED;
  return SST_OK;
}

int64_t sst_unique_workspace_bytes(int64_t n) { return sst_unique_ws_internal(n); }

int sst_unique_rows(const void* d_coors, int coor_is_i64, int64_t n, int ncols, int64_t row_stride,
                    const int64_t* h_mins, const int64_t* h_extents, int invalid_if_negative, uint32_t* d_perm,
                    int32_t* d_inverse, int32_t* d_offsets, uint64_t* d_ukeys, int32_t* d_num_unique,
                    void* d_workspace, void* stream) {
  if (n < 0 || !h_mins || !h_extents || !d_offsets || !d_num_unique) return SST_ERR_ARG;
  if (n > 0 && (!d_coors || !d_inverse || !d_workspace)) return SST_ERR_ARG;
  if (n >= (int64_t)1 << 31) return SST_ERR_UNSUPPORTED;
  hipStream_t st = (hipStream_t)stream;
  pack_params pp;
  const int bits = fill_pack_params(ncols, h_mins, h_extents, invalid_if_negative, &pp);
  if (bits < 0) return bits;
  const int64_t nn = n > 0 ? n : 1;
  sst_carver cv(d_workspace);
  uint64_t* ka = cv.take<uint64_t>(nn);
  uint64_t* kb = cv.take<uint64_t>(nn);
  void* rest = (void*)cv.take<char>(0);
  if (n > 0) {
    const int grid = sst_grid_1d(n, 256);
    if (coor_is_i64)
      hipLaunchKernelGGL(pack_keys_k<int64_t>, dim3(grid), dim3(256), 0, st, (const int64_t*)d_coors, n, row_stride,
                         pp, ka);
    else
      hipLaunchKernelGGL(pack_keys_k<int32_t>, dim3(grid), dim3(256), 0, st, (const int32_t*)d_coors, n, row_stride,
                         pp, ka);
    SST_LAUNCH_CHECK();
  }
  return sst_unique_keys_internal(ka, kb, n, bits, d_perm, d_inverse, d_offsets, d_ukeys, d_num_unique, rest, st);
}

int sst_unpack_keys(const uint64_t* d_ukeys, int64_t m, int ncols, const int64_t* h_mins, const int64_t* h_extents,
                    void* d_rows_out, int out_is_i64, int64_t out_stride, int out_col0, void* stream) {
  if (m < 0 || !h_mins || !h_extents) return SST_ERR_ARG;
  if (m == 0) return SST_OK;
  if (!d_ukeys || !d_rows_out) return SST_ERR_ARG;
  pack_params pp;
  const int bits = fill_pack_params(ncols, h_mins, h_extents, 0, &pp);
  if (bits < 0) return bits;
  hipStream_t st = (hipStream_t)stream;
  const int grid = sst_grid_1d(m, 256);
  if (out_is_i64)
    hipLaunchKernelGGL(unpack_keys_k<int64_t>, dim3(grid), dim3(256), 0, st, d_ukeys, m, pp, (int64_t*)d_rows_out,
                       out_stride, out_col0);
  else
    hipLaunchKernelGGL(unpack_keys_k<int32_t>, dim3(grid), dim3(256), 0, st, d_ukeys, m, pp, (int32_t*)d_rows_out,
                       out_stride, out_col0);
  SST_LAUNCH_CHECK();
  return SST_OK;
}

// ... 31 lines not shown
```

### sst_amd/detectors.py

```python
import torch
from torch import nn

from . import fg_sample as FS
from . import kernels as K
from . import seg_loss
from ._head_common import cfg_get as _get
from .cluster import ClusterAssigner, HybridAssigner, SSGAssigner
from .registry import BACKBONES, MODELS, ROI_EXTRACTORS, Registry, build_backbone, build_middle_encoder, build_voxel_encoder
from .sst_ops import build_mlp, scatter_v2, unique_with_plan
from .virtual_voxel import VirtualVoxelExtractor
from .voxel import Voxelization

DETECTORS = Registry('detector')
NECKS = Registry('neck')
HEADS = Registry('head')


def build_detector(cfg, train_cfg=None, test_cfg=None):
    args = dict(cfg)
    if train_cfg is not None:
        args.setdefault('train_cfg', train_cfg)
    if test_cfg is not None:
        args.setdefault('test_cfg', test_cfg)
    return DETECTORS.build(args)
# ... 212 lines not shown
    def extract_feat(self, points, img_metas=None):
        batch_points, coors = self.voxelize(points)
        coors = coors.long()
        voxel_features, voxel_coors, voxel2point_inds = self.voxel_encoder(batch_points, coors, return_inv=True)
        voxel_info = self.middle_encoder(voxel_features, voxel_coors)
        if isinstance(voxel_info, dict):
            voxel_info.setdefault('batch_size', len(points))
        x = self.backbone(voxel_info)[0]
        padding = -1
        dropped = isinstance(voxel_info, dict) and 'shuffle_inds' in voxel_info
        feats = x['voxel_feats'] if not dropped else \
            self.reorder(x['voxel_feats'], voxel_info['shuffle_inds'], voxel_info['voxel_keep_inds'], padding)
        self._dropped = dropped
        out = self.decode_neck(batch_points, coors, feats, voxel2point_inds, padding, all_valid=not dropped)
        if self.use_multiscale_features:
            return out, coors, batch_points, x['decoder_features']
        return out, coors, batch_points

    def forward(self, points, img_metas=None):
        points = self.preprocess(points)
        res = self.extract_feat(points, img_metas)
        (feats, valid), pts_coors, batch_points = res[0], res[1], res[2]
        decoder_features = res[3] if self.use_multiscale_features else None
        if self._dropped:
            batch_points, pts_coors = batch_points[valid], pts_coors[valid]
        seg_logits, vote_preds = self.segmentation_head(feats)
        return dict(seg_points=batch_points, seg_logits=seg_logits, seg_vote_preds=vote_preds,
                    offsets=self.segmentation_head.decode_vote_targets(vote_preds), seg_feats=feats,
                    batch_idx=pts_coors[:, 0], decoder_features=decoder_features)

    simple_test = forward

    def forward_train(self, points, img_metas, gt_bboxes_3d, gt_labels_3d, as_subsegmentor=False):
        points = self.preprocess(points)
        labels, vote_targets, vote_mask = self.segmentation_head.get_targets(points, gt_bboxes_3d, gt_labels_3d)
        res = self.extract_feat(points, img_metas)
        (feats, valid), pts_coors, batch_points = res[0], res[1], res[2]
        decoder_features = res[3] if self.use_multiscale_features else None
        if self._dropped:
            batch_points, pts_coors = batch_points[valid], pts_coors[valid]
            labels, vote_targets, vote_mask = labels[valid], vote_targets[valid], vote_mask[valid]
        assert feats.size(0) == labels.size(0)
        losses, preds = self.segmentation_head.forward_train(feats, img_metas, labels, vote_targets, vote_mask,
                                                             return_preds=True)
        if not as_subsegmentor:
            return losses
        return dict(seg_points=batch_points, seg_logits=preds['seg_logits'], seg_vote_preds=preds['vote_preds'],
                    offsets=self.segmentation_head.decode_vote_targets(preds['vote_preds']), seg_feats=feats,
                    batch_idx=pts_coors[:, 0], losses=losses, decoder_features=decoder_features)


@DETECTORS.register_module()
class DynamicVoxelNet(nn.Module):

    def __init__(self, voxel_layer, voxel_encoder, middle_encoder, backbone, neck=None, bbox_head=None, train_cfg=None,
                 test_cfg=None, pretrained=None, init_cfg=None):
        super().__init__()
        self.voxel_layer = Voxelization(**voxel_layer)
        self.voxel_encoder = build_voxel_encoder(voxel_encoder)
        self.middle_encoder = build_middle_encoder(middle_encoder)
        self.backbone = build_backbone(backbone)
        self.train_cfg, self.test_cfg = train_cfg, test_cfg
        self.unbuilt = {k: v for k, v in dict(neck=neck, bbox_head=bbox_head).items() if v is not None}
        self.fused_index = True
        self._planner = None

    with_neck = False

    @torch.no_grad()
    def voxelize(self, points):
        return self.voxel_layer.voxelize_batch(points)

    def _frame_planner(self, batch_size):
        from .frame_plan import FramePlanner
        from .sst_input_layer import SSTInputLayerV2
        from .voxel_encoder import DynamicVFE
        if not getattr(self, 'fused_index', True):
            return None
        planner = self.__dict__.get('_planner')
        if planner is None:
            ok = (type(self.voxel_encoder) is DynamicVFE and type(self.middle_encoder) is SSTInputLayerV2
                  and isinstance(self.voxel_layer, Voxelization) and hasattr(self.voxel_encoder, '_grid_zyx'))
            planner = FramePlanner(self.voxel_layer, self.voxel_encoder, self.middle_encoder) if ok else False
            self.__dict__['_planner'] = planner
        return planner if (planner and planner.supported(batch_size)) else None

    def prepare(self, points, overlap=False, ready_event=None):
        if len(points) == 0:
            return None
        planner = DynamicVoxelNet._frame_planner(self, len(points))
        if planner is None:
            return None
        if overlap and not any(p.is_cuda for p in points):
            return planner.build_overlapped_from_host(points, next(self.parameters()).device)
        if not all(p.is_cuda for p in points):
            return None
        return planner.build_overlapped(points, ready_event) if overlap else planner.build(points)

    def voxel_info(self, points, prepared=None):
        plan = prepared if prepared is not None else DynamicVoxelNet.prepare(self, points)
        if plan is not None:
            voxel_features, _ = self.voxel_encoder(plan.points, plan.coors, scatter_plan=plan)
            return plan.finalize(voxel_features, self.middle_encoder)
        voxels, coors = self.voxelize(points)
        voxel_features, feature_coors = self.voxel_encoder(voxels, coors)
        return self.middle_encoder(voxel_features, feature_coors, len(points))

    def extract_feat(self, points, img_metas=None, prepared=None):
        x = self.backbone(self.voxel_info(points, prepared))
        if self.with_neck:
            x = self.neck(x)
        return x

    def extract_voxel_feats(self, points, img_metas=None, prepared=None):
        info = self.voxel_info(points, prepared)
        return self.backbone.forward_voxels(info), info['voxel_coors']

    forward = extract_feat

    def attach_heads(self):
        if 'bbox_head' not in self.unbuilt:
            raise RuntimeError(f'{type(self).__name__}.attach_heads: the config has no bbox_head')
        if 'neck' in self.unbuilt:
            self.neck = build_neck(self.unbuilt['neck'])
            self.with_neck = True
        head = build_head(dict(self.unbuilt['bbox_head'], train_cfg=self.train_cfg, test_cfg=self.test_cfg))
        if hasattr(head, 'attach_network'):
            head.attach_network()
        self.bbox_head = head
        return self

    def _require_heads(self, what):
        if getattr(self, 'bbox_head', None) is None:
            raise NotImplementedError(f'{type(self).__name__}.{what}: the box head, its losses and target assignment are not built '
                                      '- call attach_heads() first (the detector parks the neck\'s and the head\'s configs in '
                                      '`unbuilt` until then)')

    def forward_train(self, points, img_metas, gt_bboxes_3d, gt_labels_3d, gt_bboxes_ignore=None):
        self._require_heads('forward_train')
        x = self.extract_feat(points, img_metas)
        outs = self.bbox_head(x)
        return self.bbox_head.loss(*outs, gt_bboxes_3d, gt_labels_3d, img_metas, gt_bboxes_ignore=gt_bboxes_ignore)

    def simple_test(self, points, img_metas, imgs=None, rescale=False):
        self._require_heads('simple_test')
        x = self.extract_feat(points, img_metas)
        outs = self.bbox_head(x)
        bbox_list = self.bbox_head.get_bboxes(*outs, img_metas, rescale=rescale)
        return [bbox3d2result(bboxes, scores, labels) for bboxes, scores, labels in bbox_list]

    def aug_test(self, *args, **kwargs):
        raise NotImplementedError(f'{type(self).__name__}.aug_test: test-time augmentation is not built')

    def losses(self, *args, **kwargs):
        raise NotImplementedError('the box head, its losses and target assignment are outside the hot path (SURVEY.md section 8)')


@DETECTORS.register_module()
class DynamicCenterPoint(DynamicVoxelNet):

    def forward_train(self, points, img_metas, gt_bboxes_3d, gt_labels_3d, gt_bboxes_ignore=None):
        self._require_heads('forward_train')
        x = self.extract_feat(points, img_metas)
        outs = self.bbox_head(x)
        return self.bbox_head.loss(gt_bboxes_3d, gt_labels_3d, outs)

    def simple_test(self, points, img_metas, imgs=None, rescale=False):
        self._require_heads('simple_test')
        x = self.extract_feat(points, img_metas)
        outs = self.bbox_head(x)
        bbox_list = self.bbox_head.get_bboxes(outs, img_metas, rescale=rescale)
        return [bbox3d2result(bboxes, scores, labels) for bboxes, scores, labels in bbox_list]


def install_fused_extract_feat(detector_cls):
    def extract_feat(self, points, img_metas=None):
        x = self.backbone(DynamicVoxelNet.voxel_info(self, points))
        if getattr(self, 'with_neck', False):
            x = self.neck(x)
        return x

    extract_feat.__doc__ = 'Extract features from points (sst_amd: fused index plan in front of the backbone).'
    detector_cls.extract_feat = extract_feat
    return detector_cls


# ... 317 lines not shown
```

### sst_amd/frame_plan.py

```python
import torch

from . import _lib
from . import kernels as K


class FramePlan(object):

    def __init__(self):
        self.want_pos_rows = True

    def reduce(self, feats, mode):
        return K.segment_reduce(feats, self.groups, mode, group_index=self.gidx, inverse=self.coors_map,
                                m_limit=self.d_counts[0:1])

    def raw_max(self, feats, scale_shift=None):
        return K._segment_reduce_fwd(feats, self.groups.perm, self.groups.offsets, self.gidx.numel(), K.REDUCE['max'], True,
                                     self.gidx, self.d_counts[0:1], self.groups, scale_shift)

    def group_sum(self, part):
        dg = self.reduce(part, 'sum')
        m = getattr(self, 'num_voxels', None)
        if m is None:
            m = int(self.d_counts[0].item())
        if m < dg.size(0):
            dg[m:].zero_()
        return K.add_group_rows_to_row0(dg, part, self.groups, self.dropped_gidx)

    @property
    def voxel_coors(self):
        return self.vcoors

    def _release_count_slot(self):
        home, slot = self.__dict__.pop('_slot_home', None), (self.__dict__.pop('h_counts', None), self.__dict__.pop('counts_ready', None))
        if home is not None and slot[0] is not None and len(home) < 64:
            home.append(slot)

    def __del__(self):
        try:
            if '_slot_home' in self.__dict__:
                self.counts_ready.synchronize()
                self._release_count_slot()
        except Exception:
            pass

    def finalize(self, voxel_feats, input_layer, feat_dim=None):
        counts = self.__dict__.get('_counts')
        if counts is None:
            self.counts_ready.synchronize()
            counts = self._counts = self.h_counts.tolist()
            self._release_count_slot()
        m, m_keep, n_win, t_max = counts[0], counts[1], (counts[2], counts[3]), (counts[4], counts[5])
        self.num_voxels, self.num_kept = m, m_keep
        dev = voxel_feats.device
        feat_index = self.feat_index[:m_keep]
        from .sst_input_layer import VoxelInfo
        info = VoxelInfo({'voxel_feats': GatherRows.apply(voxel_feats, feat_index, self.feat_index_i32[:m_keep]),
                          'voxel_coors': self.out_coors[:m_keep], 'voxel_keep_inds': feat_index})
        cap = self.max_tokens_cap
        tok0 = torch.arange(m_keep, dtype=torch.int32, device=dev)
        toks = (tok0, self.tok1)
        winoffs = (self.winoff0, self.winoff1)
        dim = voxel_feats.size(1) if feat_dim is None else feat_dim
        table = input_layer.pos_table_cached(dim, voxel_feats.dtype, dev)
        for i in range(2):
            info[f'sra_plan_shift{i}'] = K.WindowPlan(toks[i], winoffs[i], n_win[i], m_keep,
                                                      min(cap, max(1, t_max[i])), rows_in_window_order=(i == 0))
            info[f'pos_index_shift{i}'] = (self.posidx0, self.posidx1)[i][:m_keep]
        info['pos_table'] = table
        info['batch_size'] = self.batch_size
        info.defer([f'pos_embed_shift{i}' for i in range(2)], lambda d: d.update(
            {f'pos_embed_shift{i}': K.gather_rows(d['pos_table'], d[f'pos_index_shift{i}']) for i in range(2)}))
        if input_layer.reference_outputs or input_layer.debug:
            input_layer.defer_reference_entries_of_kept(info)
            if input_layer.shuffle_voxels:
                info.defer(['shuffle_inds'], lambda d, _m=m, _dev=dev: d.update(
                    shuffle_inds=torch.arange(_m, dtype=torch.int64, device=_dev)))
        return info


class GatherRows(torch.autograd.Function):

    @staticmethod
    def forward(ctx, src, index_i64, index_i32):
        ctx.save_for_backward(index_i32)
        ctx.rows = src.size(0)
        return K.gather_rows(src.contiguous(), index_i32)

    @staticmethod
    def backward(ctx, grad):
        (idx,) = ctx.saved_tensors
        out = torch.zeros((ctx.rows, grad.size(1)), dtype=grad.dtype, device=grad.device)
        K.scatter_rows(grad.contiguous(), idx, out)
        return out, None, None


class FramePlanner(object):

    def __init__(self, voxel_layer, voxel_encoder, input_layer):
        self.voxel_layer, self.vfe, self.layer = voxel_layer, voxel_encoder, input_layer
        self.grid_zyx = [int(g) for g in voxel_encoder._grid_zyx()]
        sx, sy, sz = input_layer.sparse_shape
        self.window = [int(w) for w in input_layer._window_shape3()]
        self._ok = ([sz, sy, sx] == self.grid_zyx and input_layer.window_major
                    and self.window[0] * self.window[1] * self.window[2] <= 512)

    def supported(self, batch_size):
        cells = batch_size * self.grid_zyx[0] * self.grid_zyx[1] * self.grid_zyx[2]
        return self._ok and 1 <= batch_size <= 64 and cells <= (1 << 28)

    def build_overlapped(self, points_list, ready_event=None, points_complete=False):
        dev = points_list[0].device
        main = torch.cuda.current_stream(dev)
        side = self.__dict__.get('_side_stream')
        if side is None or side.device != dev:
            side = self._side_stream = torch.cuda.Stream(device=dev, priority=-1)
        if ready_event is None and not points_complete:
            ready_event = torch.cuda.Event()
            ready_event.record(main)
        if ready_event is not None:
            side.wait_event(ready_event)
        with torch.cuda.stream(side):
            plan = self.build(points_list)
            done = torch.cuda.Event()
            done.record(side)
        seen = set()

        def mark(v, depth=0):
            if isinstance(v, torch.Tensor):
                if v.is_cuda and v.untyped_storage().data_ptr() not in seen:
                    seen.add(v.untyped_storage().data_ptr())
                    v.record_stream(main)
            elif isinstance(v, (list, tuple)):
                for u in v:
                    mark(u, depth + 1)
            elif isinstance(v, dict):
                for u in v.values():
                    mark(u, depth + 1)
            elif depth < 3 and not isinstance(v, (torch.cuda.Event, torch.cuda.Stream, type, str, int, float)) and v is not None:
                for u in list(getattr(v, '__dict__', {}).values()) + [getattr(v, a, None) for a in getattr(type(v), '__slots__', ())]:
                    mark(u, depth + 1)
        mark(plan)
        main.wait_event(done)
        plan.overlapped = True
        return plan

    def build_overlapped_from_host(self, host_points, device):
        device = torch.device(device)
        if device.index is None:
            device = torch.device('cuda', torch.cuda.current_device())
        side = self.__dict__.get('_side_stream')
        if side is None or side.device != device:
            side = self._side_stream = torch.cuda.Stream(device=device, priority=-1)
        main = torch.cuda.current_stream(device)
        with torch.cuda.stream(side):
            dev_points = [p.to(device, non_blocking=True) for p in host_points]
            copied = torch.cuda.Event()
            copied.record(side)
        for p in dev_points:
            p.record_stream(main)
        plan = self.build_overlapped(dev_points, copied)
        plan.points_list = dev_points
        return plan

    @torch.no_grad()
    def build(self, points_list):
        lib = _lib.load()
        layer, vfe = self.layer, self.vfe
        layer.set_drop_info()
        bsz = len(points_list)
        points, coors = self.voxel_layer.voxelize_batch(points_list)
        n = coors.size(0)
        dev = coors.device
        gz, gy, gx = self.grid_zyx
        plan = FramePlan()
        plan.points, plan.coors, plan.n_points = points, coors, n
        plan.batch_size = bsz
        groups = K.unique_rows(coors, [0, -1, -1, -1], [bsz, gz + 1, gy + 1, gx + 1], invalid_if_negative=2,
                               defer_count=True)
        plan.groups = groups
        n_up = max(n, 1)
        plan.n_upper = n_up

        def e32(k):
            return torch.empty(k, dtype=torch.int32, device=dev)

        plan.vcoors = torch.empty((n_up, 4), dtype=torch.int32, device=dev)
        plan.gidx, plan.coors_map = e32(n_up), e32(n_up)
        plan.d_counts = e32(8)
        plan.dropped_gidx = e32(bsz)
        grid = e32(bsz * gz * gy * gx)
        rc = lib.sst_frame_voxels_i32(_lib.ptr(groups.ukeys), _lib.ptr(groups.inverse), _lib.ptr(groups.num), n, bsz, _lib.i32array(self.grid_zyx),
                                      1 if vfe.reference_compat else 0, _lib.ptr(plan.vcoors), _lib.ptr(plan.gidx),
                                      _lib.ptr(plan.coors_map), _lib.ptr(grid), _lib.ptr(plan.d_counts),
                                      _lib.ptr(plan.dropped_gidx), _lib.stream_ptr())
        _lib.check(rc, 'sst_frame_voxels_i32')
        plan.coors_map = plan.coors_map[:n]
        _, levels = layer._levels()
        flat = []
        for (cap, lo, hi) in levels:
            flat += [int(cap), int(lo), int(min(hi, 2 ** 31 - 1))]
        plan.max_tokens_cap = max(l[0] for l in levels)
        n_win = bsz * int(lib.sst_frame_windows_per_sample(_lib.i32array(self.grid_zyx), _lib.i32array(self.window)))
        plan.feat_index = torch.empty(n_up, dtype=torch.int64, device=dev)
        plan.feat_index_i32 = e32(n_up)
        plan.out_coors = torch.empty((n_up, 4), dtype=torch.int64, device=dev)
        plan.tok1, plan.posidx0, plan.posidx1 = e32(n_up), e32(n_up), e32(n_up)
        plan.winoff0, plan.winoff1 = e32(n_win + 1), e32(n_win + 1)
        seed = int(torch.randint(1, 2 ** 31 - 1, (1,)).item()) if layer.shuffle_voxels else 0
        ws = _lib.workspace(lib.sst_window_plan_workspace_bytes(n_up, n_win), dev)
        rc = lib.sst_window_plan_i32(_lib.ptr(plan.vcoors), _lib.ptr(grid), n_up, bsz, _lib.i32array(self.grid_zyx),
                                     _lib.i32array(self.window), _lib.i32array(flat), len(levels), seed,
                                     _lib.ptr(plan.feat_index), _lib.ptr(plan.feat_index_i32), _lib.ptr(plan.out_coors),
                                     _lib.ptr(plan.tok1),
                                     _lib.ptr(plan.winoff0), _lib.ptr(plan.winoff1), _lib.ptr(plan.posidx0),
                                     _lib.ptr(plan.posidx1), _lib.ptr(plan.d_counts), _lib.ptr(ws), _lib.stream_ptr())
        _lib.check(rc, 'sst_window_plan_i32')
        plan._slot_home = self._free_count_slots()
        plan.h_counts, plan.counts_ready = plan._slot_home.pop() if plan._slot_home else (
            torch.empty(8, dtype=torch.int32, pin_memory=True), torch.cuda.Event())
        plan.h_counts.copy_(plan.d_counts, non_blocking=True)
        plan.counts_ready.record()
        return plan

    def _free_count_slots(self):
        slots = self.__dict__.get('_count_slots')
        if slots is None:
            slots = self._count_slots = []
        return slots
```

### sst_amd/kernels.py

```python
import math

import os

import torch
from torch.autograd import Function

from . import _lib

REDUCE = {'sum': 0, 'mean': 1, 'avg': 1, 'max': 2}


_CONSTANTS = {}


def const_tensor(values, device, dtype=torch.float32):
    key = (tuple(float(v) for v in values), str(device), dtype)
    t = _CONSTANTS.get(key)
    if t is None:
        t = torch.tensor([float(v) for v in values], dtype=dtype).to(device)
        _CONSTANTS[key] = t
    return t


def voxel_grid(voxel_size, coors_range):
    import ctypes
    g = (ctypes.c_int32 * 3)()
    _lib.load().sst_dynamic_voxelize_grid(_lib.farray(voxel_size), _lib.farray(coors_range), g)
    return [int(g[0]), int(g[1]), int(g[2])]


def dynamic_voxelize(points, voxel_size, coors_range, coors=None, batch_idx=-1):
    if points.dtype != torch.float32:
        raise RuntimeError('sst_amd.dynamic_voxelize: points must be float32')
    _lib.require_cuda(points)
    n = points.size(0)
    ncol = 4 if batch_idx >= 0 else 3
    if coors is None:
        coors = torch.empty((n, ncol), dtype=torch.int32, device=points.device)
    else:
        _lib.require_cuda(coors)
        if coors.dtype != torch.int32 or coors.size(0) != n or coors.size(1) != ncol:
            raise RuntimeError('sst_amd.dynamic_voxelize: coors must be int32 [N,%d]' % ncol)
    rc = _lib.load().sst_dynamic_voxelize_f32(
        _lib.ptr(points), n, points.stride(0), _lib.farray(voxel_size), _lib.farray(coors_range),
        _lib.ptr(coors), coors.stride(0) if n > 0 else ncol, ncol - 3, batch_idx, _lib.stream_ptr())
    _lib.check(rc, 'sst_dynamic_voxelize_f32')
    return coors


def exclusive_scan_i32(x):
    _lib.require_cuda(x)
    assert x.dtype == torch.int32 and x.dim() == 1
    n = x.numel()
    lib = _lib.load()
    out = torch.empty_like(x)
    total = torch.zeros(1, dtype=torch.int32, device=x.device)
    ws = _lib.workspace(lib.sst_scan_workspace_bytes(n), x.device)
    rc = lib.sst_exclusive_scan_i32(_lib.ptr(x), _lib.ptr(out), n, _lib.ptr(total), _lib.ptr(ws), _lib.stream_ptr())
    _lib.check(rc, 'sst_exclusive_scan_i32')
    return out, total


def sort_pairs_u64(keys, key_bits):
    _lib.require_cuda(keys)
    assert keys.dtype == torch.int64 and keys.dim() == 1
    n = keys.numel()
    lib = _lib.load()
    kin = keys.clone()
    kout = torch.empty_like(keys)
    perm = torch.empty(n, dtype=torch.int32, device=keys.device)
    ws = _lib.workspace(lib.sst_sort_workspace_bytes(n), keys.device)
    rc = lib.sst_sort_pairs_u64(_lib.ptr(kin), _lib.ptr(kout), _lib.ptr(perm), n, int(key_bits), _lib.ptr(ws),
                                _lib.stream_ptr())
    _lib.check(rc, 'sst_sort_pairs_u64')
    return kout, perm


class UniquePlan(object):
    __slots__ = ('n', 'm', 'num', 'perm', 'inverse', 'offsets', 'ukeys', 'mins', 'extents', 'ncols', 'has_invalid_group',
                 'scratch', 'native')

    def counts(self):
        return self.offsets[1:self.m + 1] - self.offsets[:self.m]


def unique_rows(coors, mins=None, extents=None, invalid_if_negative=False, defer_count=False):
    _lib.require_cuda(coors)
    if coors.dtype not in (torch.int32, torch.int64) or coors.dim() != 2:
        raise RuntimeError('sst_amd.unique_rows: coors must be a 2-D int32/int64 tensor')
    n, k = coors.shape
    dev = coors.device
    lib = _lib.load()
    if n > 0 and (mins is None or extents is None):
        lo = coors.amin(0)
        hi = coors.amax(0)
        lohi = torch.stack([lo, hi]).tolist()
        mins = [int(v) for v in lohi[0]]
        if int(invalid_if_negative) == 1:
            mins = [max(v, 0) for v in mins]
        extents = [max(int(h) - int(l) + 1, 1) for l, h in zip(mins, lohi[1])]
    elif n == 0:
        mins = [0] * k
        extents = [1] * k
    plan = UniquePlan()
    plan.n, plan.ncols = n, k
    plan.native = True
    plan.mins, plan.extents = list(mins), list(extents)
    plan.perm = torch.empty(max(n, 1), dtype=torch.int32, device=dev)
    plan.inverse = torch.empty(max(n, 1), dtype=torch.int32, device=dev)
    plan.offsets = torch.empty(n + 1, dtype=torch.int32, device=dev)
    plan.ukeys = torch.empty(max(n, 1), dtype=torch.int64, device=dev)
    num = torch.zeros(1, dtype=torch.int32, device=dev)
    ws = _lib.workspace(lib.sst_unique_workspace_bytes(n), dev)
    rc = lib.sst_unique_rows(_lib.ptr(coors), 1 if coors.dtype == torch.int64 else 0, n, k,
                             coors.stride(0) if n > 0 else k, _lib.i64array(mins), _lib.i64array(extents),
                             int(invalid_if_negative), _lib.ptr(plan.perm), _lib.ptr(plan.inverse),
                             _lib.ptr(plan.offsets), _lib.ptr(plan.ukeys), _lib.ptr(num), _lib.ptr(ws),
                             _lib.stream_ptr())
    _lib.check(rc, 'sst_unique_rows')
    plan.num = num
    if defer_count:
        plan.m = None
    else:
        plan.m = int(num.item())
    plan.inverse = plan.inverse[:n]
    plan.perm = plan.perm[:n]
    return plan


def unpack_unique_rows(plan, dtype, first=0, count=None, out_cols=None, col0=0, out=None):
    lib = _lib.load()
    m = plan.m - first if count is None else count
    k = plan.ncols
    dev = plan.ukeys.device
    width = k if out_cols is None else out_cols
    if out is None:
        out = torch.empty((m, width), dtype=dtype, device=dev)
    if m > 0:
        keys = plan.ukeys[first:first + m]
        rc = lib.sst_unpack_keys(_lib.ptr(keys), m, k, _lib.i64array(plan.mins), _lib.i64array(plan.extents),
                                 _lib.ptr(out), 1 if dtype == torch.int64 else 0, out.stride(0), col0,
                                 _lib.stream_ptr())
        _lib.check(rc, 'sst_unpack_keys')
    return out


def _long_work_list(plan, n, m, c, dev):
    cache = getattr(plan, 'scratch', None)
    if cache is None:
        cache = plan.scratch = {}
    key = ('work', _lib.stream_ptr().value, (c + 3) // 4)
    buf = cache.get(key)
    need = int(_lib.load().sst_segment_reduce_work_words(n, max(int(m), int(getattr(plan, 'm', 0) or 0)), c))
    if buf is None or buf.numel() < need:
        buf = cache[key] = torch.zeros(need, dtype=torch.int32, device=dev)
    return buf


def _segment_reduce_fwd(feats, perm, offsets, m, mode, want_argmax, group_index=None, m_limit=None, plan=None,
                        scale_shift=None):
    n, c = feats.shape
    out = torch.empty((m, c), dtype=torch.float32, device=feats.device)
    argmax = torch.empty((m, c), dtype=torch.int32, device=feats.device) if want_argmax else None
    work = _long_work_list(plan, n, m, c, feats.device) if (plan is not None and n > 0
                                                      and os.environ.get('SST_SEG_WORK', '1') != '0') else None
    rc = _lib.load().sst_segment_reduce_fwd_work_f32(_lib.ptr(feats), n, c, _lib.ptr(perm), _lib.ptr(offsets),
                                                     _lib.ptr(group_index), m, mode, _lib.ptr(out), _lib.ptr(argmax),
                                                     _lib.ptr(m_limit), _lib.ptr(work), 0 if work is None else work.numel(),
                                                     _lib.ptr(scale_shift[0]) if scale_shift is not None else None,
                                                     _lib.ptr(scale_shift[1]) if scale_shift is not None else None,
                                                     _lib.stream_ptr())
    _lib.check(rc, 'sst_segment_reduce_fwd_work_f32')
    return out, argmax


def _long_group_scratch(plan, n, m, c, dev):
    cache = getattr(plan, 'scratch', None)
    if cache is None:
        cache = plan.scratch = {}
    buf = cache.get((n, m, c))
    if buf is None:
        buf = cache[(n, m, c)] = torch.zeros(int(_lib.load().sst_segment_long_scratch_bytes(n, m, c)), dtype=torch.uint8,
                                             device=dev)
    return buf


def _long_group_applies(n, m, c, inverse, group_index, m_limit):
    cv = c // 4 if c % 4 == 0 else c
    return (group_index is None and m_limit is None and inverse is not None and m > 0 and n >= 8 * m and c <= 256
            and (256 % cv == 0 or cv * min(32, 256 // cv) <= 256) and os.environ.get('SST_SEG_LONG', '1') != '0')


class SegmentReduce(Function):

    @staticmethod
    def forward(ctx, feats, perm, offsets, inverse, m, mode, inverse_shift, group_index=None, m_limit=None, plan=None):
        if feats.dtype != torch.float32:
            raise RuntimeError('sst_amd: features must be float32')
        feats = feats.contiguous()
        _lib.require_cuda(feats, perm, offsets)
        n, c = feats.shape
        if plan is not None and _long_group_applies(n, m, c, inverse, group_index, m_limit) \
                and (c % 4 != 0 or feats.data_ptr() % 16 == 0):
            if getattr(plan, 'native', False):
                out = torch.empty((m, c), dtype=torch.float32, device=feats.device)
                argmax = torch.empty((m, c), dtype=torch.int32, device=feats.device) if mode == 2 else None
            else:
                out = torch.zeros((m, c), dtype=torch.float32, device=feats.device)
                argmax = torch.full((m, c), n, dtype=torch.int32, device=feats.device) if mode == 2 else None
            scratch = _long_group_scratch(plan, n, m, c, feats.device)
            rc = _lib.load().sst_segment_reduce_long_f32(_lib.ptr(feats), n, c, _lib.ptr(perm), _lib.ptr(inverse),
                                                         int(inverse_shift), _lib.ptr(offsets), m, mode, _lib.ptr(scratch),
                                                         _lib.ptr(out), _lib.ptr(argmax), _lib.stream_ptr())
            _lib.check(rc, 'sst_segment_reduce_long_f32')
        else:
            out, argmax = _segment_reduce_fwd(feats, perm, offsets, m, mode, mode == 2, group_index, m_limit, plan)
        ctx.mode, ctx.m, ctx.shift = mode, m, inverse_shift
        ctx.shape = feats.shape
        ctx.has_gidx = group_index is not None
        ctx.m_limit = m_limit
        ctx.save_for_backward(offsets, inverse, argmax if argmax is not None else offsets,
                              group_index if group_index is not None else offsets)
        return out

    @staticmethod
    def backward(ctx, grad_out):
        offsets, inverse, argmax, gidx = ctx.saved_tensors
        n, c = ctx.shape
        grad_out = grad_out.contiguous()
        grad_feats = torch.empty((n, c), dtype=torch.float32, device=grad_out.device)
        rc = _lib.load().sst_segment_reduce_bwd_f32(
            _lib.ptr(grad_out), ctx.m, c, _lib.ptr(inverse), ctx.shift, _lib.ptr(offsets),
            _lib.ptr(gidx) if ctx.has_gidx else None, _lib.ptr(argmax) if ctx.mode == 2 else None, n, ctx.mode,
# ... 468 lines not shown
```

### sst_amd/vfe_fused.py

```python
import torch
from torch import nn
from torch.autograd.function import Function

from . import _lib
from . import kernels as K
from .dense import weight_bias_grad
from .norm import bn_prepare

EPI_BIAS = 0


def _x6_linear(x, w_ptr, ldw, trans_w, m, k, n, name):
    y = torch.empty((m, n), dtype=torch.float32, device=x.device)
    rc = _lib.load().sst_tall_linear_epi_f32x6(_lib.ptr(x), x.stride(0), w_ptr, ldw, int(trans_w), None, m, k, n, EPI_BIAS,
                                               None, None, 0, _lib.ptr(y), n, _lib.stream_ptr())
    _lib.check(rc, name)
    return y


def _float_ptr(t, offset_elems=0):
    import ctypes
    return ctypes.c_void_p(t.data_ptr() + 4 * offset_elems)


def fused_vfe2_ok(encoder, x, plan):
    layers = getattr(encoder, 'vfe_layers', None)
    if layers is None or len(layers) != 2 or encoder.mode != 'max' or encoder.return_point_feats:
        return False
    l0, l1 = layers
    for l in (l0, l1):
        relu = isinstance(getattr(l, 'act', None), nn.ReLU) if hasattr(l, 'act') else True
        if not (isinstance(l.norm, nn.BatchNorm1d) and l.norm.weight is not None and l.norm.bias is not None
                and relu and getattr(l, 'dropout', None) is None and l.linear.bias is None):
            return False
    return (x.is_cuda and x.dtype == torch.float32 and x.dim() == 2 and x.size(0) > 0 and not x.requires_grad
            and x.size(1) == l0.linear.in_features and x.size(1) <= 16 and l0.linear.out_features == 64
            and l1.linear.in_features == 128 and l1.linear.out_features in (64, 128)
            and l0.linear.weight.is_contiguous() and l1.linear.weight.is_contiguous()
            and hasattr(plan, 'raw_max') and hasattr(plan, 'group_sum')
            and getattr(plan, 'num_voxels', 1) != 0)


class FusedVFE2(Function):

    @staticmethod
    def forward(ctx, x, w0, g0, b0, w1, g1, b1, plan, bn0, bn1):
        lib = _lib.load()
        x = x.contiguous()
        n, k = x.shape
        c0, c1 = w0.size(0), w1.size(0)
        dev = x.device
        st = _lib.stream_ptr
        y0 = torch.empty((n, c0), dtype=torch.float32, device=dev)
        ws = _lib.workspace(lib.sst_bn_workspace_bytes(n, c0), dev)
        rc = lib.sst_vfe_linear_moments_f32(_lib.ptr(x), x.stride(0), n, k, _lib.ptr(w0), w0.stride(0), c0, _lib.ptr(y0), c0,
                                            _lib.ptr(ws), st())
        _lib.check(rc, 'sst_vfe_linear_moments_f32')
        prep0, bs0, cnt0, sync0 = bn_prepare(bn0, y0, partials=ws)
        pf0 = torch.empty((n, c0), dtype=torch.float32, device=dev)
        rc = lib.sst_bn_act_fwd_f32(_lib.ptr(y0), n, c0, c0, _lib.ptr(prep0[2]), _lib.ptr(prep0[3]), 1, _lib.ptr(pf0), c0, st())
        _lib.check(rc, 'sst_bn_act_fwd_f32')
        pooled0, arg0 = plan.raw_max(pf0)
        rows = pooled0.size(0)
        t = _x6_linear(pooled0, _float_ptr(w1, c0), w1.stride(0), 0, rows, c0, c1, 'sst_tall_linear_epi_f32x6 (pooled half)')
        y1 = torch.empty((n, c1), dtype=torch.float32, device=dev)
        index = plan.coors_map
        rc = lib.sst_tall_linear_add_rows_f32x6(_lib.ptr(pf0), c0, _lib.ptr(w1), w1.stride(0), n, c0, c1, _lib.ptr(t), c1,
                                                _lib.ptr(index), _lib.ptr(y1), c1, st())
        _lib.check(rc, 'sst_tall_linear_add_rows_f32x6')
        prep1, bs1, cnt1, sync1 = bn_prepare(bn1, y1)
        out, arg1 = plan.raw_max(y1, scale_shift=(prep1[2], prep1[3]))
        ctx.save_for_backward(x, y0, pf0, pooled0, arg0, y1, arg1, prep0, prep1, w0, w1, index)
        ctx.plan = plan
        ctx.cfg = ((bs0, cnt0, sync0), (bs1, cnt1, sync1))
        return out

    @staticmethod
    def backward(ctx, dout):
        from torch import distributed as dist
        x, y0, pf0, pooled0, arg0, y1, arg1, prep0, prep1, w0, w1, index = ctx.saved_tensors
        plan = ctx.plan
        (bs0, cnt0, sync0), (bs1, cnt1, sync1) = ctx.cfg
        lib = _lib.load()
        st = _lib.stream_ptr
        n, k = x.shape
        c0, c1 = w0.size(0), w1.size(0)
        dev = x.device
        dout = dout.contiguous()

        def bn_pool_bwd(dy, xin, c, prep, arg, dpool, batch_stats, count, sync):
            sums = torch.empty((2, c), dtype=torch.float32, device=dev)
            ws = _lib.workspace(lib.sst_bn_workspace_bytes(n, c), dev)
            rc = lib.sst_bn_act_pool_bwd_reduce_f32(_lib.ptr(dy), _lib.ptr(xin), n, c, c, c, _lib.ptr(prep[0]), _lib.ptr(prep[1]),
                                                    _lib.ptr(prep[2]), _lib.ptr(prep[3]), 1, _lib.ptr(index), _lib.ptr(arg),
                                                    _lib.ptr(dpool), dpool.stride(0), _lib.ptr(sums[0]), _lib.ptr(sums[1]),
                                                    _lib.ptr(ws), st())
            _lib.check(rc, 'sst_bn_act_pool_bwd_reduce_f32')
            total = sums
            if sync and batch_stats:
                total = sums.clone()
                dist.all_reduce(total, async_op=False)
            dx = torch.empty((n, c), dtype=torch.float32, device=dev)
            rc = lib.sst_bn_act_pool_bwd_apply_f32(_lib.ptr(dy), _lib.ptr(xin), n, c, c, c, _lib.ptr(prep[0]), _lib.ptr(prep[1]),
                                                   _lib.ptr(prep[2]), _lib.ptr(prep[3]), _lib.ptr(total[0]), _lib.ptr(total[1]),
                                                   (1.0 / count) if batch_stats else 0.0, 1, _lib.ptr(index), _lib.ptr(arg),
                                                   _lib.ptr(dpool), dpool.stride(0), _lib.ptr(dx), c, st())
            _lib.check(rc, 'sst_bn_act_pool_bwd_apply_f32')
            return dx, sums

        dy1, sums1 = bn_pool_bwd(None, y1, c1, prep1, arg1, dout, bs1, cnt1, sync1)
        dt = plan.group_sum(dy1)
        m = getattr(plan, 'num_voxels', None)
        if m is None:
            m = int(plan.d_counts[0].item())
        dw1a, _ = weight_bias_grad(dy1, pf0, False)
        dw1b, _ = weight_bias_grad(dt[:m], pooled0[:m], False)
        dw1 = torch.cat([dw1a, dw1b], dim=1)
        dpf0 = _x6_linear(dy1, _lib.ptr(w1), w1.stride(0), 1, n, c1, c0, 'sst_tall_linear_epi_f32x6 (d point half)')
        dpooled0 = _x6_linear(dt, _float_ptr(w1, c0), w1.stride(0), 1, dt.size(0), c1, c0,
                              'sst_tall_linear_epi_f32x6 (d pooled half)')
        dy0, sums0 = bn_pool_bwd(dpf0, y0, c0, prep0, arg0, dpooled0, bs0, cnt0, sync0)
        dw0, _ = weight_bias_grad(dy0, x, False)
        return None, dw0, sums0[1], sums0[0], dw1, sums1[1], sums1[0], None, None, None


def fused_vfe2(encoder, x, plan):
    l0, l1 = encoder.vfe_layers
    return FusedVFE2.apply(x, l0.linear.weight, l0.norm.weight, l0.norm.bias, l1.linear.weight, l1.norm.weight, l1.norm.bias,
                           plan, l0.norm, l1.norm)


class UniquePlanAdapter(object):

    def __init__(self, plan):
        self.plan = plan
        self.coors_map = plan.inverse
        self.num_voxels = plan.m

    def raw_max(self, feats, scale_shift=None):
        p = self.plan
        return K._segment_reduce_fwd(feats, p.perm, p.offsets, p.m, K.REDUCE['max'], True, None, None, p, scale_shift)

    def group_sum(self, part):
        return K.segment_reduce(part, self.plan, 'sum')
```

Baseline: 100.6.

## Fuse first VFE layer BN backward with weight gradient and add kept-row planning

```diff
diff --git a/include/sst_amd.h b/include/sst_amd.h
--- a/include/sst_amd.h
+++ b/include/sst_amd.h
@@ -23,6 +23,7 @@
 void sst_dynamic_voxelize_grid(const float voxel_size[3], const float coors_range[6], int32_t grid_xyz[3]);
 
 int64_t sst_scan_workspace_bytes(int64_t n);
+int64_t sst_scan_one_launch_max(void);
 int sst_exclusive_scan_i32(const int32_t* d_in, int32_t* d_out, int64_t n, int32_t* d_total,
                            void* d_workspace, void* stream);
 
@@ -101,6 +102,13 @@
                         uint32_t seed, int64_t* d_feat_index, int32_t* d_feat_index32, int64_t* d_out_coors,
                         int32_t* d_tok1, int32_t* d_winoff0, int32_t* d_winoff1, int32_t* d_posidx0, int32_t* d_posidx1,
                         int32_t* d_counts, void* d_workspace, void* stream);
+int sst_window_plan_rows_i32(const int32_t* d_vcoors, const int32_t* d_grid, int64_t n_upper, int batch_size,
+                             const int32_t grid_zyx[3], const int32_t window_shape[3], const int32_t* h_levels, int n_levels,
+                             uint32_t seed, int64_t* d_feat_index, int32_t* d_feat_index32, int64_t* d_out_coors,
+                             int32_t* d_tok1, int32_t* d_winoff0, int32_t* d_winoff1, int32_t* d_posidx0,
+                             int32_t* d_posidx1, int32_t* d_counts, const int32_t* d_gidx, const int32_t* d_coors_map,
+                             int64_t n_points, int32_t* d_kept_gidx, int32_t* d_row_of_point, int32_t* d_tok0,
+                             void* d_workspace, void* stream);
 
 int sst_sra_attn_fwd_f32(const float* d_q, const float* d_k, const float* d_v, int64_t ldq, int64_t ldk,
                          int64_t ldv, const int32_t* d_tok, const int32_t* d_winoff, int64_t n_windows,
@@ -279,6 +287,13 @@
                                   const float* d_coef_a, const float* d_coef_b, float coef_scale, int act,
                                   const int32_t* d_group, const int32_t* d_arg, const float* d_dpool, int64_t ldp, float* d_dx,
                                   int64_t lddx, void* stream);
+int64_t sst_bn_act_pool_bwd_dw_workspace_bytes(int64_t n);
+int sst_bn_act_pool_bwd_dw_f32(const float* d_dy, const float* d_x, int64_t n, int c, int64_t lddy, int64_t ldx,
+                               const float* d_mean, const float* d_invstd, const float* d_scale, const float* d_shift,
+                               const float* d_coef_a, const float* d_coef_b, float coef_scale, int act,
+                               const int32_t* d_group, const int32_t* d_arg, const float* d_dpool, int64_t ldp,
+                               const float* d_in, int64_t ldin, int k, float* d_dw, int64_t lddw, void* d_workspace,
+                               void* stream);
 int sst_bn_act_res_fwd_f32(const float* d_x, int64_t n, int c, int64_t ldx, const float* d_res, int64_t ldr,
                            const float* d_scale, const float* d_shift, int act, float* d_y, int64_t ldy, void* stream);
 int sst_bn_act_res_bwd_reduce_f32(const float* d_dy, const float* d_x, const float* d_res, int64_t n, int c,
diff --git a/sst_amd/_lib.py b/sst_amd/_lib.py
--- a/sst_amd/_lib.py
+++ b/sst_amd/_lib.py
@@ -208,6 +208,7 @@
     'sst_dynamic_voxelize_f32': (c_i32, [c_ptr, c_i64, c_i64, c_ptr, c_ptr, c_ptr, c_i64, c_i32, c_i32, c_ptr]),
     'sst_dynamic_voxelize_grid': (None, [c_ptr, c_ptr, c_ptr]),
     'sst_scan_workspace_bytes': (c_i64, [c_i64]),
+    'sst_scan_one_launch_max': (c_i64, []),
     'sst_exclusive_scan_i32': (c_i32, [c_ptr, c_ptr, c_i64, c_ptr, c_ptr, c_ptr]),
     'sst_sort_workspace_bytes': (c_i64, [c_i64]),
     'sst_sort_pairs_u64': (c_i32, [c_ptr, c_ptr, c_ptr, c_i64, c_i32, c_ptr, c_ptr]),
@@ -249,6 +250,10 @@
                                                c_ptr, c_ptr, c_ptr, c_i64, c_ptr, c_ptr, c_ptr, c_ptr]),
     'sst_bn_act_pool_bwd_apply_f32': (c_i32, [c_ptr, c_ptr, c_i64, c_i32, c_i64, c_i64, c_ptr, c_ptr, c_ptr, c_ptr, c_ptr,
                                               c_ptr, c_f32, c_i32, c_ptr, c_ptr, c_ptr, c_i64, c_ptr, c_i64, c_ptr]),
+    'sst_bn_act_pool_bwd_dw_workspace_bytes': (c_i64, [c_i64]),
+    'sst_bn_act_pool_bwd_dw_f32': (c_i32, [c_ptr, c_ptr, c_i64, c_i32, c_i64, c_i64, c_ptr, c_ptr, c_ptr, c_ptr, c_ptr,
+                                           c_ptr, c_f32, c_i32, c_ptr, c_ptr, c_ptr, c_i64, c_ptr, c_i64, c_i32, c_ptr, c_i64,
+                                           c_ptr, c_ptr]),
     'sst_tall_linear_add_rows_f32x6': (c_i32, [c_ptr, c_i64, c_ptr, c_i64, c_i64, c_i32, c_i32, c_ptr, c_i64, c_ptr, c_ptr,
                                                c_i64, c_ptr]),
     'sst_segment_long_scratch_bytes': (c_i64, [c_i64, c_i64, c_i32]),
@@ -268,6 +273,8 @@
                                      c_ptr, c_ptr, c_ptr]),
     'sst_window_plan_workspace_bytes': (c_i64, [c_i64, c_i64]),
     'sst_window_plan_i32': (c_i32, [c_ptr, c_ptr, c_i64, c_i32, c_ptr, c_ptr, c_ptr, c_i32, ctypes.c_uint32] + [c_ptr] * 11),
+    'sst_window_plan_rows_i32': (c_i32, [c_ptr, c_ptr, c_i64, c_i32, c_ptr, c_ptr, c_ptr, c_i32, ctypes.c_uint32] + [c_ptr] * 11
+                                 + [c_i64] + [c_ptr] * 5),
     'sst_sra_attn_fwd_f32': (c_i32, [c_ptr, c_ptr, c_ptr, c_i64, c_i64, c_i64, c_ptr, c_ptr, c_i64, c_i32,
                                      c_f32, c_i32, c_i32, c_ptr, c_i64, c_ptr, c_ptr]),
     'sst_sra_attn_bwd_f32': (c_i32, [c_ptr] * 6 + [c_i64] * 5 + [c_ptr, c_ptr, c_i64, c_i64, c_i32, c_f32,
diff --git a/sst_amd/csrc/bn.hip b/sst_amd/csrc/bn.hip
--- a/sst_amd/csrc/bn.hip
+++ b/sst_amd/csrc/bn.hip
@@ -240,6 +240,93 @@
   }
 }
 
+constexpr int kDwC = 64, kDwK = 16;
+__global__ __launch_bounds__(kBnThreads) void bn_act_bwd_dw_k(const float* __restrict__ dy, const float* __restrict__ x,
+                                                             int64_t n, int64_t lddy, int64_t ldx,
+                                                             const float* __restrict__ mean,
+                                                             const float* __restrict__ invstd,
+                                                             const float* __restrict__ scale,
+                                                             const float* __restrict__ shift,
+                                                             const float* __restrict__ ca, const float* __restrict__ cb,
+                                                             float coef_scale, int act, const float* __restrict__ xin,
+                                                             int64_t ldin, int k, int64_t rows_per_block,
+                                                             float* __restrict__ partial, const bn_pool_grad pg) {
+  __shared__ float red[4][kDwC * kDwK];
+  constexpr int c = kDwC, rpi = kBnThreads / (kDwC / 4);
+  const int ry = threadIdx.x >> 4, cx = threadIdx.x & 15;
+  const int64_t beg = (int64_t)blockIdx.x * rows_per_block;
+  const int64_t end = beg + rows_per_block < n ? beg + rows_per_block : n;
+  const float4 sc = *(const float4*)(scale + cx * 4);
+  const float4 sh = *(const float4*)(shift + cx * 4);
+  const float4 mu = *(const float4*)(mean + cx * 4);
+  const float4 is = *(const float4*)(invstd + cx * 4);
+  float4 a = *(const float4*)(ca + cx * 4);
+  float4 b = *(const float4*)(cb + cx * 4);
+  a.x *= coef_scale, a.y *= coef_scale, a.z *= coef_scale, a.w *= coef_scale;
+  b.x *= coef_scale, b.y *= coef_scale, b.z *= coef_scale, b.w *= coef_scale;
+  float acc[kDwK][4];
+#pragma unroll
+  for (int kk = 0; kk < kDwK; ++kk) acc[kk][0] = acc[kk][1] = acc[kk][2] = acc[kk][3] = 0.f;
+  for (int64_t row = beg + ry; row < end; row += rpi) {
+    const float4 v = *(const float4*)(x + row * ldx + cx * 4);
+    float4 g = make_float4(0.f, 0.f, 0.f, 0.f);
+    if (dy != nullptr) g = *(const float4*)(dy + row * lddy + cx * 4);
+    if (pg.group != nullptr) {
+      const float4 sp = bn_pool_part(pg, row, c, cx);
+      g.x += sp.x, g.y += sp.y, g.z += sp.z, g.w += sp.w;
+    }
+    if (act) {
+      g.x = (v.x * sc.x + sh.x) > 0.f ? g.x : 0.f;
+      g.y = (v.y * sc.y + sh.y) > 0.f ? g.y : 0.f;
+      g.z = (v.z * sc.z + sh.z) > 0.f ? g.z : 0.f;
+      g.w = (v.w * sc.w + sh.w) > 0.f ? g.w : 0.f;
+    }
+    float4 o;
+    o.x = sc.x * (g.x - a.x - (v.x - mu.x) * is.x * b.x);
+    o.y = sc.y * (g.y - a.y - (v.y - mu.y) * is.y * b.y);
+    o.z = sc.z * (g.z - a.z - (v.z - mu.z) * is.z * b.z);
+    o.w = sc.w * (g.w - a.w - (v.w - mu.w) * is.w * b.w);
+    const float* xr = xin + row * ldin;
+#pragma unroll
+    for (int kk = 0; kk < kDwK; ++kk) {
+      const float xv = kk < k ? xr[kk] : 0.f;
+      acc[kk][0] = fmaf(o.x, xv, acc[kk][0]), acc[kk][1] = fmaf(o.y, xv, acc[kk][1]);
+      acc[kk][2] = fmaf(o.z, xv, acc[kk][2]), acc[kk][3] = fmaf(o.w, xv, acc[kk][3]);
+    }
+  }
+  const int wave = threadIdx.x >> 6, lane = threadIdx.x & 63;
+#pragma unroll
+  for (int kk = 0; kk < kDwK; ++kk)
+#pragma unroll
+    for (int q = 0; q < 4; ++q) {
+      float t = acc[kk][q];
+      t += __shfl_xor(t, 16);
+      t += __shfl_xor(t, 32);
+      if (lane < 16) red[wave][(cx * 4 + q) * kDwK + kk] = t;
+    }
+  __syncthreads();
+  float* dst = partial + (int64_t)blockIdx.x * (kDwC * kDwK);
+  for (int i = threadIdx.x; i < kDwC * kDwK; i += kBnThreads) dst[i] = (red[0][i] + red[1][i]) + (red[2][i] + red[3][i]);
+}
+
+__global__ __launch_bounds__(1024) void dw_finish_k(const float* __restrict__ partial, int nb, int k,
+                                                    float* __restrict__ dw, int64_t lddw) {
+  __shared__ double r[32][33];
+  const int cx = threadIdx.x & 31, gy = threadIdx.x >> 5;
+  const int i = blockIdx.x * 32 + cx;
+  double s = 0.;
+  for (int b = gy; b < nb; b += 32) s += (double)partial[(int64_t)b * (kDwC * kDwK) + i];
+  r[gy][cx] = s;
+  __syncthreads();
+  if (gy == 0) {
+    double t = 0.;
+#pragma unroll
+    for (int j = 0; j < 32; ++j) t += r[j][cx];
+    const int ch = i / kDwK, kk = i - ch * kDwK;
+    if (kk < k) dw[(int64_t)ch * lddw + kk] = (float)t;
+  }
+}
+
 __global__ __launch_bounds__(kBnThreads) void vfe_linear_smallk_k(const float* __restrict__ x, int64_t ldx, int64_t n, int k,
                                                                  const float* __restrict__ w, int64_t ldw, int c,
                                                                  float* __restrict__ y, int64_t ldy, int64_t rows_per_block,
@@ -535,4 +622,39 @@
   return SST_OK;
 }
 
-}
+int64_t sst_bn_act_pool_bwd_dw_workspace_bytes(int64_t n) {
+  (void)n;
+  return (int64_t)512 * kDwC * kDwK * sizeof(float) + 256;
+}
+
+int sst_bn_act_pool_bwd_dw_f32(const float* d_dy, const float* d_x, int64_t n, int c, int64_t lddy, int64_t ldx,
+                               const float* d_mean, const float* d_invstd, const float* d_scale, const float* d_shift,
+                               const float* d_coef_a, const float* d_coef_b, float coef_scale, int act,
+                               const int32_t* d_group, const int32_t* d_arg, const float* d_dpool, int64_t ldp,
+                               const float* d_in, int64_t ldin, int k, float* d_dw, int64_t lddw, void* d_workspace,
+                               void* stream) {
+  if (n < 0 || c != kDwC || k < 1 || k > kDwK || ldx < c || (ldx & 3) || act < 0 || act > 1 || ldp < c || (ldp & 3) ||
+      ldin < k || lddw < k)
+    return SST_ERR_UNSUPPORTED;
+  if (d_dy && (lddy < c || (lddy & 3) || ((uintptr_t)d_dy & 15))) return SST_ERR_UNSUPPORTED;
+  if (!d_dw) return SST_ERR_ARG;
+  hipStream_t st = (hipStream_t)stream;
+  if (n == 0) {
+    SST_HIP(hipMemset2DAsync(d_dw, sizeof(float) * lddw, 0, sizeof(float) * k, c, st));
+    return SST_OK;
+  }
+  if (!d_x || !d_mean || !d_invstd || !d_scale || !d_shift || !d_coef_a || !d_coef_b || !d_in || !d_workspace || !d_group ||
+      !d_arg || !d_dpool || ((uintptr_t)d_x & 15) || ((uintptr_t)d_arg & 15) || ((uintptr_t)d_dpool & 15))
+    return SST_ERR_ARG;
+  int64_t rpb;
+  const int grid = moments_grid(n, &rpb);
+  float* partial = (float*)d_workspace;
+  hipLaunchKernelGGL(bn_act_bwd_dw_k, dim3(grid), dim3(kBnThreads), 0, st, d_dy, d_x, n, lddy, ldx, d_mean, d_invstd, d_scale,
+                     d_shift, d_coef_a, d_coef_b, coef_scale, act, d_in, ldin, k, rpb, partial,
+                     bn_pool_grad{d_group, d_arg, d_dpool, ldp});
+  hipLaunchKernelGGL(dw_finish_k, dim3(kDwC * kDwK / 32), dim3(1024), 0, st, partial, grid, k, d_dw, lddw);
+  SST_LAUNCH_CHECK();
+  return SST_OK;
+}
+
+}
diff --git a/sst_amd/csrc/frame_plan.hip b/sst_amd/csrc/frame_plan.hip
--- a/sst_amd/csrc/frame_plan.hip
+++ b/sst_amd/csrc/frame_plan.hip
@@ -277,8 +277,15 @@
                                                  const int32_t* __restrict__ tokbase1, int64_t* __restrict__ feat_index,
                                                  int32_t* __restrict__ feat_index32,
                                                  int64_t* __restrict__ out_coors, int32_t* __restrict__ tok1,
-                                                 int32_t* __restrict__ posidx0, int32_t* __restrict__ posidx1) {
+                                                 int32_t* __restrict__ posidx0, int32_t* __restrict__ posidx1,
+                                                 const int32_t* __restrict__ gidx, const int32_t* __restrict__ coors_map,
+                                                 int n_points, int n_upper, int32_t* __restrict__ kept_gidx,
+                                                 int32_t* __restrict__ row_of_point, int32_t* __restrict__ tok0) {
   const int m = d_counts[0];
+  if (tok0 != nullptr)
+    for (int r = blockIdx.x * blockDim.x + threadIdx.x; r < n_upper; r += gridDim.x * blockDim.x) tok0[r] = r;
+  if (kept_gidx != nullptr)
+    for (int r = d_counts[1] + blockIdx.x * blockDim.x + threadIdx.x; r < n_upper; r += gridDim.x * blockDim.x) kept_gidx[r] = -1;
   for (int v = blockIdx.x * blockDim.x + threadIdx.x; v < m; v += gridDim.x * blockDim.x) {
     if (keep[v] == 0) continue;
     const int b = vcoors[4 * v], z = vcoors[4 * v + 1], y = vcoors[4 * v + 2], x = vcoors[4 * v + 3];
@@ -295,7 +302,19 @@
     posidx0[ni] = p0;
     posidx1[ni] = p1;
     tok1[tokbase1[w1] + inner1[v]] = ni;
-  }
+    if (kept_gidx != nullptr) kept_gidx[ni] = gidx[v];
+  }
+  if (row_of_point != nullptr)
+    for (int i = blockIdx.x * blockDim.x + threadIdx.x; i < n_points; i += gridDim.x * blockDim.x) {
+      const int v = coors_map[i];
+      int row = -1;
+      if (v >= 0 && v < m && keep[v] != 0) {
+        int w0, p0;
+        fp_window_of(G, 0, vcoors[4 * v], vcoors[4 * v + 1], vcoors[4 * v + 2], vcoors[4 * v + 3], w0, p0);
+        row = tokbase0[w0] + inner0[v];
+      }
+      row_of_point[i] = row;
+    }
 }
 
 int fill_geom(fp_geom* G, int batch_size, const int32_t grid_zyx[3], const int32_t window_shape[3],
@@ -367,13 +386,16 @@
   return 4 * sst_align_up(4 * n, 256) + 4 * sst_align_up(4 * (w + 1), 256);
 }
 
-int sst_window_plan_i32(const int32_t* d_vcoors, const int32_t* d_grid, int64_t n_upper, int batch_size,
-                        const int32_t grid_zyx[3], const int32_t window_shape[3], const int32_t* h_levels, int n_levels,
-                        uint32_t seed, int64_t* d_feat_index, int32_t* d_feat_index32, int64_t* d_out_coors,
-                        int32_t* d_tok1,
-                        int32_t* d_winoff0, int32_t* d_winoff1, int32_t* d_posidx0, int32_t* d_posidx1,
-                        int32_t* d_counts, void* d_workspace, void* stream) {
+int sst_window_plan_rows_i32(const int32_t* d_vcoors, const int32_t* d_grid, int64_t n_upper, int batch_size,
+                             const int32_t grid_zyx[3], const int32_t window_shape[3], const int32_t* h_levels, int n_levels,
+                             uint32_t seed, int64_t* d_feat_index, int32_t* d_feat_index32, int64_t* d_out_coors,
+                             int32_t* d_tok1, int32_t* d_winoff0, int32_t* d_winoff1, int32_t* d_posidx0,
+                             int32_t* d_posidx1, int32_t* d_counts, const int32_t* d_gidx, const int32_t* d_coors_map,
+                             int64_t n_points, int32_t* d_kept_gidx, int32_t* d_row_of_point, int32_t* d_tok0, void* d_workspace,
+                             void* stream) {
   if (n_upper < 0 || n_levels < 1 || n_levels > 8 || !h_levels) return SST_ERR_ARG;
+  if (n_points < 0 || n_points > 0x7fffffff || (d_kept_gidx && !d_gidx) || (d_row_of_point && n_points > 0 && !d_coors_map))
+    return SST_ERR_ARG;
   fp_geom G;
   int rc = fill_geom(&G, batch_size, grid_zyx, window_shape, h_levels, n_levels);
   if (rc != SST_OK) return rc;
@@ -403,9 +425,21 @@
   hipLaunchKernelGGL(fp_window_scan_k, dim3(2), dim3(1024), 0, st, cntk0, cntk1, n_win, tokbase0, tokbase1, d_winoff0,
                      d_winoff1, d_counts);
   hipLaunchKernelGGL(fp_fill_k, dim3(sst_grid_1d(n_upper, 256)), dim3(256), 0, st, d_vcoors, d_counts, G, keep, inner0,
-                     inner1, tokbase0, tokbase1, d_feat_index, d_feat_index32, d_out_coors, d_tok1, d_posidx0, d_posidx1);
+                     inner1, tokbase0, tokbase1, d_feat_index, d_feat_index32, d_out_coors, d_tok1, d_posidx0, d_posidx1,
+                     d_gidx, d_coors_map, (int)n_points, (int)n_upper, d_kept_gidx, d_row_of_point, d_tok0);
   SST_LAUNCH_CHECK();
   return SST_OK;
 }
 
-}
+int sst_window_plan_i32(const int32_t* d_vcoors, const int32_t* d_grid, int64_t n_upper, int batch_size,
+                        const int32_t grid_zyx[3], const int32_t window_shape[3], const int32_t* h_levels, int n_levels,
+                        uint32_t seed, int64_t* d_feat_index, int32_t* d_feat_index32, int64_t* d_out_coors,
+                        int32_t* d_tok1,
+                        int32_t* d_winoff0, int32_t* d_winoff1, int32_t* d_posidx0, int32_t* d_posidx1,
+                        int32_t* d_counts, void* d_workspace, void* stream) {
+  return sst_window_plan_rows_i32(d_vcoors, d_grid, n_upper, batch_size, grid_zyx, window_shape, h_levels, n_levels, seed,
+                                  d_feat_index, d_feat_index32, d_out_coors, d_tok1, d_winoff0, d_winoff1, d_posidx0, d_posidx1,
+                                  d_counts, nullptr, nullptr, 0, nullptr, nullptr, nullptr, d_workspace, stream);
+}
+
+}
diff --git a/sst_amd/csrc/sort_scan.hip b/sst_amd/csrc/sort_scan.hip
--- a/sst_amd/csrc/sort_scan.hip
+++ b/sst_amd/csrc/sort_scan.hip
@@ -76,9 +76,62 @@
   }
 }
 
+constexpr int kScan1Threads = 1024;
+constexpr int kScan1Tile = kScan1Threads * 4;
+constexpr int64_t kScanOneLaunchMax = 262144;
+
+__device__ __forceinline__ int4 scan1_load(const int32_t* in, int i, int n) {
+  if (i + 3 < n) return *(const int4*)(in + i);
+  int4 v = make_int4(0, 0, 0, 0);
+  if (i < n) v.x = in[i];
+  if (i + 1 < n) v.y = in[i + 1];
+  if (i + 2 < n) v.z = in[i + 2];
+  return v;
+}
+
+__global__ __launch_bounds__(kScan1Threads) void scan_one_k(const int32_t* in, int32_t* out, int n,
+                                                            int32_t* __restrict__ total_out) {
+  __shared__ int wsum[2][16];
+  const int lane = threadIdx.x & 63, wave = threadIdx.x >> 6;
+  const int ntiles = (n + kScan1Tile - 1) / kScan1Tile;
+  int carry = 0;
+  int4 nxt = scan1_load(in, threadIdx.x * 4, n);
+  for (int t = 0; t < ntiles; ++t) {
+    const int i = t * kScan1Tile + threadIdx.x * 4;
+    const int4 v = nxt;
+    if (t + 1 < ntiles) nxt = scan1_load(in, i + kScan1Tile, n);
+    const int s = v.x + v.y + v.z + v.w;
+    const int incl = sst_wave_incl_scan(s);
+    if (lane == 63) wsum[t & 1][wave] = incl;
+    __syncthreads();
+    int woff = 0, tot = 0;
+#pragma unroll
+    for (int w = 0; w < 16; ++w) {
+      const int x = wsum[t & 1][w];
+      if (w < wave) woff += x;
+      tot += x;
+    }
+    const int run = carry + woff + incl - s;
+    if (i + 3 < n) {
+      *(int4*)(out + i) = make_int4(run, run + v.x, run + v.x + v.y, run + v.x + v.y + v.z);
+    } else {
+      if (i < n) out[i] = run;
+      if (i + 1 < n) out[i + 1] = run + v.x;
+      if (i + 2 < n) out[i + 2] = run + v.x + v.y;
+    }
+    carry += tot;
+  }
+  if (threadIdx.x == 0 && total_out != nullptr) *total_out = carry;
+}
+
 int scan_impl(const int32_t* d_in, int32_t* d_out, int64_t n, int32_t* d_total, void* ws, hipStream_t st) {
   if (n <= 0) {
     if (d_total) SST_HIP(hipMemsetAsync(d_total, 0, sizeof(int32_t), st));
+    return SST_OK;
+  }
+  if (n <= kScanOneLaunchMax && ((((uintptr_t)d_in) | ((uintptr_t)d_out)) & 15) == 0) {
+    hipLaunchKernelGGL(scan_one_k, dim3(1), dim3(kScan1Threads), 0, st, d_in, d_out, (int)n, d_total);
+    SST_LAUNCH_CHECK();
     return SST_OK;
   }
   const int nb = (int)sst_div_up(n, kScanTile);
@@ -369,6 +422,8 @@
 extern "C" {
 
 int64_t sst_scan_workspace_bytes(int64_t n) { return scan_ws_bytes(n); }
+
+int64_t sst_scan_one_launch_max(void) { return kScanOneLaunchMax; }
 
 int sst_exclusive_scan_i32(const int32_t* d_in, int32_t* d_out, int64_t n, int32_t* d_total, void* d_workspace,
                            void* stream) {
diff --git a/sst_amd/detectors.py b/sst_amd/detectors.py
--- a/sst_amd/detectors.py
+++ b/sst_amd/detectors.py
@@ -318,6 +318,8 @@
             ok = (type(self.voxel_encoder) is DynamicVFE and type(self.middle_encoder) is SSTInputLayerV2
                   and isinstance(self.voxel_layer, Voxelization) and hasattr(self.voxel_encoder, '_grid_zyx'))
             planner = FramePlanner(self.voxel_layer, self.voxel_encoder, self.middle_encoder) if ok else False
+            if planner:
+                planner.kept_rows = True
             self.__dict__['_planner'] = planner
         return planner if (planner and planner.supported(batch_size)) else None
 
@@ -336,8 +338,12 @@
     def voxel_info(self, points, prepared=None):
         plan = prepared if prepared is not None else DynamicVoxelNet.prepare(self, points)
         if plan is not None:
-            voxel_features, _ = self.voxel_encoder(plan.points, plan.coors, scatter_plan=plan)
-            return plan.finalize(voxel_features, self.middle_encoder)
+            plan.kept_rows_wanted, plan.kept_layout_ptr = True, None
+            try:
+                voxel_features, _ = self.voxel_encoder(plan.points, plan.coors, scatter_plan=plan)
+            finally:
+                plan.kept_rows_wanted = False
+            return plan.finalize(voxel_features, self.middle_encoder, kept_rows=plan.kept_layout_ptr is not None)
         voxels, coors = self.voxelize(points)
         voxel_features, feature_coors = self.voxel_encoder(voxels, coors)
         return self.middle_encoder(voxel_features, feature_coors, len(points))
diff --git a/sst_amd/frame_plan.py b/sst_amd/frame_plan.py
--- a/sst_amd/frame_plan.py
+++ b/sst_amd/frame_plan.py
@@ -8,6 +8,9 @@
 
     def __init__(self):
         self.want_pos_rows = True
+        self.kept_gidx = self.row_of_point = None
+        self.kept_rows_wanted = False
+        self.kept_layout_ptr = None
 
     def reduce(self, feats, mode):
         return K.segment_reduce(feats, self.groups, mode, group_index=self.gidx, inverse=self.coors_map,
@@ -16,6 +19,10 @@
     def raw_max(self, feats, scale_shift=None):
         return K._segment_reduce_fwd(feats, self.groups.perm, self.groups.offsets, self.gidx.numel(), K.REDUCE['max'], True,
                                      self.gidx, self.d_counts[0:1], self.groups, scale_shift)
+
+    def raw_max_kept(self, feats, scale_shift=None):
+        return K._segment_reduce_fwd(feats, self.groups.perm, self.groups.offsets, self.kept_gidx.numel(), K.REDUCE['max'], True,
+                                     self.kept_gidx, self.d_counts[1:2], self.groups, scale_shift)
 
     def group_sum(self, part):
         dg = self.reduce(part, 'sum')
@@ -43,7 +50,12 @@
         except Exception:
             pass
 
-    def finalize(self, voxel_feats, input_layer, feat_dim=None):
+    def finalize(self, voxel_feats, input_layer, feat_dim=None, kept_rows=False):
+        produced = self.kept_layout_ptr is not None and voxel_feats.data_ptr() == self.kept_layout_ptr \
+            and voxel_feats.size(0) == self.n_upper
+        if kept_rows != produced:
+            raise RuntimeError('sst_amd: FramePlan.finalize(kept_rows=%s) but the voxel features %s the output the encoder '
+                               'wrote in kept order for this plan' % (kept_rows, 'are' if produced else 'are not'))
         counts = self.__dict__.get('_counts')
         if counts is None:
             self.counts_ready.synchronize()
@@ -54,10 +66,14 @@
         dev = voxel_feats.device
         feat_index = self.feat_index[:m_keep]
         from .sst_input_layer import VoxelInfo
-        info = VoxelInfo({'voxel_feats': GatherRows.apply(voxel_feats, feat_index, self.feat_index_i32[:m_keep]),
+        if kept_rows:
+            kept_feats = KeptRows.apply(voxel_feats, m_keep)
+        else:
+            kept_feats = GatherRows.apply(voxel_feats, feat_index, self.feat_index_i32[:m_keep])
+        info = VoxelInfo({'voxel_feats': kept_feats,
                           'voxel_coors': self.out_coors[:m_keep], 'voxel_keep_inds': feat_index})
         cap = self.max_tokens_cap
-        tok0 = torch.arange(m_keep, dtype=torch.int32, device=dev)
+        tok0 = self.tok0[:m_keep]
         toks = (tok0, self.tok1)
         winoffs = (self.winoff0, self.winoff1)
         dim = voxel_feats.size(1) if feat_dim is None else feat_dim
@@ -94,10 +110,25 @@
         return out, None, None
 
 
+class KeptRows(torch.autograd.Function):
+
+    @staticmethod
+    def forward(ctx, feats, m_keep):
+        ctx.rows = feats.size(0)
+        return feats[:m_keep]
+
+    @staticmethod
+    def backward(ctx, grad):
+        out = torch.empty((ctx.rows, grad.size(1)), dtype=grad.dtype, device=grad.device)
+        out[:grad.size(0)].copy_(grad)
+        return out, None
+
+
 class FramePlanner(object):
 
     def __init__(self, voxel_layer, voxel_encoder, input_layer):
         self.voxel_layer, self.vfe, self.layer = voxel_layer, voxel_encoder, input_layer
+        self.kept_rows = False
         self.grid_zyx = [int(g) for g in voxel_encoder._grid_zyx()]
         sx, sy, sz = input_layer.sparse_shape
         self.window = [int(w) for w in input_layer._window_shape3()]
@@ -208,13 +239,19 @@
         plan.winoff0, plan.winoff1 = e32(n_win + 1), e32(n_win + 1)
         seed = int(torch.randint(1, 2 ** 31 - 1, (1,)).item()) if layer.shuffle_voxels else 0
         ws = _lib.workspace(lib.sst_window_plan_workspace_bytes(n_up, n_win), dev)
-        rc = lib.sst_window_plan_i32(_lib.ptr(plan.vcoors), _lib.ptr(grid), n_up, bsz, _lib.i32array(self.grid_zyx),
-                                     _lib.i32array(self.window), _lib.i32array(flat), len(levels), seed,
-                                     _lib.ptr(plan.feat_index), _lib.ptr(plan.feat_index_i32), _lib.ptr(plan.out_coors),
-                                     _lib.ptr(plan.tok1),
-                                     _lib.ptr(plan.winoff0), _lib.ptr(plan.winoff1), _lib.ptr(plan.posidx0),
-                                     _lib.ptr(plan.posidx1), _lib.ptr(plan.d_counts), _lib.ptr(ws), _lib.stream_ptr())
-        _lib.check(rc, 'sst_window_plan_i32')
+        plan.tok0 = e32(n_up)
+        if self.kept_rows:
+            plan.kept_gidx, plan.row_of_point = e32(n_up), e32(n_up)[:n]
+        groups.work_cache = self.__dict__.setdefault('_seg_work_cache', {})
+        rc = lib.sst_window_plan_rows_i32(_lib.ptr(plan.vcoors), _lib.ptr(grid), n_up, bsz, _lib.i32array(self.grid_zyx),
+                                          _lib.i32array(self.window), _lib.i32array(flat), len(levels), seed,
+                                          _lib.ptr(plan.feat_index), _lib.ptr(plan.feat_index_i32), _lib.ptr(plan.out_coors),
+                                          _lib.ptr(plan.tok1),
+                                          _lib.ptr(plan.winoff0), _lib.ptr(plan.winoff1), _lib.ptr(plan.posidx0),
+                                          _lib.ptr(plan.posidx1), _lib.ptr(plan.d_counts), _lib.ptr(plan.gidx),
+                                          _lib.ptr(plan.coors_map), n, _lib.ptr(plan.kept_gidx), _lib.ptr(plan.row_of_point),
+                                          _lib.ptr(plan.tok0), _lib.ptr(ws), _lib.stream_ptr())
+        _lib.check(rc, 'sst_window_plan_rows_i32')
         plan._slot_home = self._free_count_slots()
         plan.h_counts, plan.counts_ready = plan._slot_home.pop() if plan._slot_home else (
             torch.empty(8, dtype=torch.int32, pin_memory=True), torch.cuda.Event())
diff --git a/sst_amd/kernels.py b/sst_amd/kernels.py
--- a/sst_amd/kernels.py
+++ b/sst_amd/kernels.py
@@ -78,7 +78,8 @@
 
 class UniquePlan(object):
     __slots__ = ('n', 'm', 'num', 'perm', 'inverse', 'offsets', 'ukeys', 'mins', 'extents', 'ncols', 'has_invalid_group',
-                 'scratch', 'native')
+                 'scratch', 'native',
+                 'work_cache')
 
     def counts(self):
         return self.offsets[1:self.m + 1] - self.offsets[:self.m]
@@ -146,9 +147,11 @@
 
 
 def _long_work_list(plan, n, m, c, dev):
-    cache = getattr(plan, 'scratch', None)
+    cache = getattr(plan, 'work_cache', None)
     if cache is None:
-        cache = plan.scratch = {}
+        cache = getattr(plan, 'scratch', None)
+        if cache is None:
+            cache = plan.scratch = {}
     key = ('work', _lib.stream_ptr().value, (c + 3) // 4)
     buf = cache.get(key)
     need = int(_lib.load().sst_segment_reduce_work_words(n, max(int(m), int(getattr(plan, 'm', 0) or 0)), c))
diff --git a/sst_amd/vfe_fused.py b/sst_amd/vfe_fused.py
--- a/sst_amd/vfe_fused.py
+++ b/sst_amd/vfe_fused.py
@@ -69,8 +69,13 @@
                                                 _lib.ptr(index), _lib.ptr(y1), c1, st())
         _lib.check(rc, 'sst_tall_linear_add_rows_f32x6')
         prep1, bs1, cnt1, sync1 = bn_prepare(bn1, y1)
-        out, arg1 = plan.raw_max(y1, scale_shift=(prep1[2], prep1[3]))
-        ctx.save_for_backward(x, y0, pf0, pooled0, arg0, y1, arg1, prep0, prep1, w0, w1, index)
+        index1 = index
+        if _kept_rows(plan):
+            out, arg1 = plan.raw_max_kept(y1, scale_shift=(prep1[2], prep1[3]))
+            index1 = plan.row_of_point
+        else:
+            out, arg1 = plan.raw_max(y1, scale_shift=(prep1[2], prep1[3]))
+        ctx.save_for_backward(x, y0, pf0, pooled0, arg0, y1, arg1, prep0, prep1, w0, w1, index, index1)
         ctx.plan = plan
         ctx.cfg = ((bs0, cnt0, sync0), (bs1, cnt1, sync1))
         return out
@@ -78,7 +83,7 @@
     @staticmethod
     def backward(ctx, dout):
         from torch import distributed as dist
-        x, y0, pf0, pooled0, arg0, y1, arg1, prep0, prep1, w0, w1, index = ctx.saved_tensors
+        x, y0, pf0, pooled0, arg0, y1, arg1, prep0, prep1, w0, w1, index, index1 = ctx.saved_tensors
         plan = ctx.plan
         (bs0, cnt0, sync0), (bs1, cnt1, sync1) = ctx.cfg
         lib = _lib.load()
@@ -88,7 +93,7 @@
         dev = x.device
         dout = dout.contiguous()
 
-        def bn_pool_bwd(dy, xin, c, prep, arg, dpool, batch_stats, count, sync):
+        def bn_pool_bwd(dy, xin, c, prep, arg, dpool, index, batch_stats, count, sync, dw_of=None):
             sums = torch.empty((2, c), dtype=torch.float32, device=dev)
             ws = _lib.workspace(lib.sst_bn_workspace_bytes(n, c), dev)
             rc = lib.sst_bn_act_pool_bwd_reduce_f32(_lib.ptr(dy), _lib.ptr(xin), n, c, c, c, _lib.ptr(prep[0]), _lib.ptr(prep[1]),
@@ -100,6 +105,16 @@
             if sync and batch_stats:
                 total = sums.clone()
                 dist.all_reduce(total, async_op=False)
+            if dw_of is not None:
+                dw = torch.empty((c, dw_of.size(1)), dtype=torch.float32, device=dev)
+                ws = _lib.workspace(lib.sst_bn_act_pool_bwd_dw_workspace_bytes(n), dev)
+                rc = lib.sst_bn_act_pool_bwd_dw_f32(_lib.ptr(dy), _lib.ptr(xin), n, c, c, c, _lib.ptr(prep[0]), _lib.ptr(prep[1]),
+                                                    _lib.ptr(prep[2]), _lib.ptr(prep[3]), _lib.ptr(total[0]), _lib.ptr(total[1]),
+                                                    (1.0 / count) if batch_stats else 0.0, 1, _lib.ptr(index), _lib.ptr(arg),
+                                                    _lib.ptr(dpool), dpool.stride(0), _lib.ptr(dw_of), dw_of.stride(0),
+                                                    dw_of.size(1), _lib.ptr(dw), dw.stride(0), _lib.ptr(ws), st())
+                _lib.check(rc, 'sst_bn_act_pool_bwd_dw_f32')
+                return dw, sums
             dx = torch.empty((n, c), dtype=torch.float32, device=dev)
             rc = lib.sst_bn_act_pool_bwd_apply_f32(_lib.ptr(dy), _lib.ptr(xin), n, c, c, c, _lib.ptr(prep[0]), _lib.ptr(prep[1]),
                                                    _lib.ptr(prep[2]), _lib.ptr(prep[3]), _lib.ptr(total[0]), _lib.ptr(total[1]),
@@ -108,7 +123,7 @@
             _lib.check(rc, 'sst_bn_act_pool_bwd_apply_f32')
             return dx, sums
 
-        dy1, sums1 = bn_pool_bwd(None, y1, c1, prep1, arg1, dout, bs1, cnt1, sync1)
+        dy1, sums1 = bn_pool_bwd(None, y1, c1, prep1, arg1, dout, index1, bs1, cnt1, sync1)
         dt = plan.group_sum(dy1)
         m = getattr(plan, 'num_voxels', None)
         if m is None:
@@ -119,15 +134,21 @@
         dpf0 = _x6_linear(dy1, _lib.ptr(w1), w1.stride(0), 1, n, c1, c0, 'sst_tall_linear_epi_f32x6 (d point half)')
         dpooled0 = _x6_linear(dt, _float_ptr(w1, c0), w1.stride(0), 1, dt.size(0), c1, c0,
                               'sst_tall_linear_epi_f32x6 (d pooled half)')
-        dy0, sums0 = bn_pool_bwd(dpf0, y0, c0, prep0, arg0, dpooled0, bs0, cnt0, sync0)
-        dw0, _ = weight_bias_grad(dy0, x, False)
+        dw0, sums0 = bn_pool_bwd(dpf0, y0, c0, prep0, arg0, dpooled0, index, bs0, cnt0, sync0, dw_of=x)
         return None, dw0, sums0[1], sums0[0], dw1, sums1[1], sums1[0], None, None, None
+
+
+def _kept_rows(plan):
+    return bool(getattr(plan, 'kept_rows_wanted', False)) and getattr(plan, 'kept_gidx', None) is not None
 
 
 def fused_vfe2(encoder, x, plan):
     l0, l1 = encoder.vfe_layers
-    return FusedVFE2.apply(x, l0.linear.weight, l0.norm.weight, l0.norm.bias, l1.linear.weight, l1.norm.weight, l1.norm.bias,
-                           plan, l0.norm, l1.norm)
+    out = FusedVFE2.apply(x, l0.linear.weight, l0.norm.weight, l0.norm.bias, l1.linear.weight, l1.norm.weight, l1.norm.bias,
+                          plan, l0.norm, l1.norm)
+    if _kept_rows(plan):
+        plan.kept_layout_ptr = out.data_ptr()
+    return out
 
 
 class UniquePlanAdapter(object):
```

Result: no change. 101.4 (median of 6 runs) (+0.7%).
